# DenisKolodin/safe_gossip

Measured on AMD Instinct MI355X. Metric: node-rumor updates/sec (whole node) + % HBM roofline; rounds-to-full-spread, higher is better.
Workload: dtype u64

## Files before the change

include/safe_gossip.h:

```cpp
#ifndef SAFE_GOSSIP_H
#define SAFE_GOSSIP_H

#include <stdint.h>

#ifdef __cplusplus
extern "C" {
#endif

typedef enum {
    GS_OK = 0,
    GS_ERR_NO_PEERS = 1,
    GS_ERR_ALREADY_STARTED = 2,
    GS_ERR_SIG_FAILURE = 3,
    GS_ERR_IO = 4,
    GS_ERR_SERIALISATION = 5,
    GS_ERR_INVALID_ARGUMENT = -1,
    GS_ERR_UNSUPPORTED = -2,
    GS_ERR_HIP = -3,
    GS_ERR_OUT_OF_MEMORY = -4,
    GS_ERR_DEVICE_LIMIT = -5
} gs_status;

typedef enum { GS_SCHED_2P = 0, GS_SCHED_SEQ = 1 } gs_schedule;

typedef struct {
    uint32_t n_nodes;
    uint32_t n_rumors;
    uint64_t seed;
    uint32_t epoch;
    uint8_t counter_max;
    uint8_t max_c_rounds;
    uint8_t max_rounds;
    uint8_t schedule;
    int32_t device;
    uint32_t churn;
    uint32_t drop_push;
    uint32_t drop_pull;
    uint32_t rumor_slice;
    uint32_t reserved1[3];
} gs_config;

typedef struct {
    uint64_t rounds;
    uint64_t empty_pull_sent;
    uint64_t empty_push_sent;
    uint64_t full_message_sent;
    uint64_t full_message_received;
} gs_statistics_t;

typedef enum { GS_REDUCE_SUM = 0, GS_REDUCE_MIN = 1, GS_REDUCE_MAX = 2 } gs_reduce_op;

typedef struct {
    uint32_t round;
    uint32_t any_live;
} gs_round_report;

typedef struct gs_engine gs_engine;

#define GS_ABI_VERSION 2u
uint32_t    gs_abi_version(void);
const char *gs_build_id(void);

gs_status   gs_create(const gs_config *cfg, gs_engine **out);
void        gs_destroy(gs_engine *e);
gs_status   gs_get_params(const gs_engine *e, uint8_t out[3]);

gs_status   gs_send_new(gs_engine *e, uint32_t node, uint32_t rumor);

gs_status   gs_set_params(gs_engine *e, const uint8_t params[3]);

gs_status   gs_next_round(gs_engine *e, gs_round_report *report);

gs_status   gs_statistics(gs_engine *e, uint32_t node, gs_statistics_t *out);
gs_status   gs_statistics_all(gs_engine *e, uint64_t *out );
gs_status   gs_statistics_reduce(gs_engine *e, gs_reduce_op op, gs_statistics_t *out);
gs_status   gs_messages(gs_engine *e, uint32_t node, uint64_t *words );
gs_status   gs_known_all(gs_engine *e, uint64_t *words );
gs_status   gs_known_counts(gs_engine *e, uint64_t *known_total, uint64_t *nodes_complete);
gs_status   gs_known_counts_min(gs_engine *e, uint32_t min_known, uint64_t *known_total,
                                uint64_t *nodes_complete);
gs_status   gs_known_popcounts(gs_engine *e, uint32_t *counts);

gs_status   gs_dump_state(gs_engine *e, uint16_t *out);
gs_status   gs_dump_records(gs_engine *e, uint16_t *rec, uint32_t *psize);
gs_status   gs_state_digest(gs_engine *e, uint64_t *out);
gs_status   gs_state_digest_part(gs_engine *e, uint32_t rumor_lo, uint32_t words, uint64_t *dpart);
gs_status   gs_digest_finish(gs_engine *e, const uint64_t *dpart, uint32_t words, const uint64_t *stats,
                             uint64_t *out);

gs_status   gs_clear(gs_engine *e, uint32_t epoch);
gs_status   gs_sync(gs_engine *e);
uint32_t    gs_round(const gs_engine *e);

float       gs_last_round_kernel_ms(gs_engine *e);
void        gs_set_timing(gs_engine *e, int enable);
int32_t     gs_round_kernel_times(gs_engine *e, float *out_ms, uint32_t max);
double      gs_round_kernel_bytes(const gs_engine *e);
const char *gs_round_kernel_name(const gs_engine *e);
gs_status   gs_round_traffic(gs_engine *e, double *bytes_per_launch, uint32_t *launches);

gs_status   gs_shard_create(const gs_config *cfg, uint32_t rank, uint32_t world, gs_engine **out);
gs_status   gs_shard_create_parts(const gs_config *cfg, uint32_t rank, uint32_t world, uint32_t parts,
                                  gs_engine **out);
gs_status   gs_shard_info(const gs_engine *e, uint32_t info[14]);
gs_status   gs_shard_plan_info(const gs_config *cfg, uint32_t rank, uint32_t world, uint32_t parts,
                               uint32_t info[14]);
gs_status   gs_shard_bind(gs_engine *e, void *sendA0, void *sendA1, void *recvA0, void *recvA1,
                          void *sendB, void *recvB);
gs_status   gs_shard_round_part(gs_engine *e, uint32_t part);
gs_status   gs_shard_pull(gs_engine *e);
uint64_t    gs_stream(const gs_engine *e);
int         gs_device(const gs_engine *e);

gs_status   gs_slice_bind(gs_engine *e, void *buf0, void *buf1, void *buf2, void *obs);
gs_status   gs_slice_apply(gs_engine *e, uint32_t which);
gs_status   gs_slice_defer(gs_engine *e, uint32_t which);
gs_status   gs_slice_set_ext_limit(gs_engine *e, uint32_t limit);

#define GS_NET_ID_BYTES 128
typedef struct gs_net gs_net;
typedef enum { GS_NET_SLICES = 0, GS_NET_SHARDS = 1 } gs_net_mode;
gs_status   gs_net_unique_id(uint8_t id[GS_NET_ID_BYTES]);
gs_status   gs_net_create(const gs_config *cfg, gs_net_mode mode, uint32_t rank, uint32_t world, uint32_t parts,
                          const uint8_t id[GS_NET_ID_BYTES], gs_net **out);
gs_status   gs_net_create_local(const gs_config *cfg, gs_net_mode mode, uint32_t world, uint32_t parts,
                                gs_net **out);
void        gs_net_destroy(gs_net *net);
enum { GS_NET_U8 = 0, GS_NET_U32 = 1, GS_NET_U64 = 2 };
enum { GS_NET_SUM = 0, GS_NET_MIN = 1, GS_NET_MAX = 2 };
typedef struct {
    void *ctx;
    int (*alltoall)(void *ctx, const void *send, void *recv, uint64_t bytes_per_rank);
    int (*allreduce)(void *ctx, void *buf, uint64_t count, int dtype, int op);
    int (*allgather)(void *ctx, const void *send, void *recv, uint64_t bytes_per_rank);
} gs_net_collectives;
gs_status   gs_net_create_with(const gs_config *cfg, gs_net_mode mode, uint32_t rank, uint32_t world, uint32_t parts,
                               const gs_net_collectives *coll, gs_net **out);
gs_status   gs_net_send_new(gs_net *net, uint32_t node, uint32_t rumor);
gs_status   gs_net_next_round(gs_net *net, gs_round_report *report);
gs_status   gs_net_sync(gs_net *net);
gs_status   gs_net_clear(gs_net *net, uint32_t epoch);
gs_status   gs_net_known_counts(gs_net *net, uint64_t *known_total, uint64_t *nodes_complete);
gs_status   gs_net_statistics_all(gs_net *net, uint64_t *out );
gs_status   gs_net_dump_state(gs_net *net, uint16_t *out );
uint32_t    gs_net_local_engines(const gs_net *net);
gs_engine  *gs_net_engine(gs_net *net, uint32_t i);

gs_status   gs_rpc_encode(int pull, const uint8_t *msg, uint32_t msg_len, uint8_t counter, uint8_t *out,
                          uint32_t cap, uint32_t *out_len);
gs_status   gs_rpc_decode(const uint8_t *buf, uint32_t len, int *pull, uint32_t *msg_off, uint32_t *msg_len,
                          uint8_t *counter);
gs_status   gs_message_wrap(const uint8_t *payload, uint32_t len, const uint8_t signature[64], uint8_t *out,
                            uint32_t cap, uint32_t *out_len);
gs_status   gs_message_unwrap(const uint8_t *buf, uint32_t len, uint32_t *payload_off, uint32_t *payload_len,
                              uint32_t *signature_off);
gs_status   gs_set_rumor_key(gs_engine *e, uint32_t rumor, const uint8_t *key, uint32_t len);
gs_status   gs_rumor_key(const gs_engine *e, uint32_t rumor, uint8_t *out, uint32_t cap, uint32_t *len);
gs_status   gs_push_batch(gs_engine *e, uint32_t node, uint8_t *out, uint32_t cap, uint32_t *len,
                          uint32_t *count);
gs_status   gs_handle_received(gs_engine *e, uint32_t node, uint32_t peer, const uint8_t *msg,
                               uint32_t msg_len, uint8_t *out, uint32_t cap, uint32_t *out_len,
                               uint32_t *out_count);
gs_status   gs_handle_received_batch(gs_engine *e, uint32_t count, const uint32_t *nodes, const uint32_t *peers,
                                     const uint8_t *msgs, const uint32_t *off, const uint32_t *len, uint8_t *out,
                                     uint32_t cap, uint32_t *out_len, uint32_t *resp_off);

gs_status   gs_sha3_512(int device, uint32_t count, const uint8_t *data, const uint32_t *off,
                        const uint32_t *len, uint8_t *out);
gs_status   gs_ed25519_verify(int device, uint32_t count, const uint8_t *pubs, const uint8_t *sigs,
                              const uint8_t *msgs, const uint32_t *off, const uint32_t *len, uint8_t *ok);
gs_status   gs_ed25519_sign(int device, uint32_t count, const uint8_t *seeds, const uint8_t *msgs,
                            const uint32_t *off, const uint32_t *len, uint8_t *pubs, uint8_t *sigs);
gs_status   gs_handle_received_signed(gs_engine *e, uint32_t node, uint32_t peer, const uint8_t peer_key[32],
                                      const uint8_t node_seed[32], const uint8_t *msg, uint32_t msg_len,
                                      uint8_t *out, uint32_t cap, uint32_t *out_len, uint32_t *out_count);
gs_status   gs_push_batch_signed(gs_engine *e, uint32_t node, const uint8_t node_seed[32], uint8_t *out,
                                 uint32_t cap, uint32_t *len, uint32_t *count);

uint32_t    gs_peer(uint64_t seed, uint32_t epoch, uint32_t round, uint32_t node, uint32_t n);
uint32_t    gs_origin(uint64_t seed, uint32_t epoch, uint32_t rumor, uint32_t n);
uint32_t    gs_coin(uint64_t seed, uint32_t epoch, uint32_t round, uint32_t node);
uint32_t    gs_fault(uint64_t seed, uint32_t epoch, uint32_t round, uint32_t node,
// ... 9 lines not shown
```

safe_gossip_amd/__init__.py:

```python
from __future__ import annotations

import ctypes
import os
from dataclasses import dataclass
from typing import List, Optional, Sequence

import numpy as np

from .build import LIB_PATH

__all__ = [
    "Network", "Gossiper", "Statistics", "RoundReport", "GossipError", "NoPeers",
    "AlreadyStarted", "DeviceError", "derive_params", "peer_of", "origin_of", "coin_of",
    "send_messages", "load_library", "SYMBOLS", "rpc_encode", "rpc_decode", "message_wrap",
    "message_unwrap", "split_frames", "SigFailure", "sha3_512", "ed25519_sign", "ed25519_verify",
    "default_rumor_key",
]

class GossipError(Exception):

    code = None


class NoPeers(GossipError):
# ... 14 lines not shown
class DeviceError(GossipError):
    """Engine-side failure (no library, no GPU, HIP error, device limit)."""


_ERRORS = {1: NoPeers, 2: AlreadyStarted, 3: SigFailure}

class _Config(ctypes.Structure):
    _fields_ = [
        ("n_nodes", ctypes.c_uint32), ("n_rumors", ctypes.c_uint32),
        ("seed", ctypes.c_uint64), ("epoch", ctypes.c_uint32),
        ("counter_max", ctypes.c_uint8), ("max_c_rounds", ctypes.c_uint8),
        ("max_rounds", ctypes.c_uint8), ("schedule", ctypes.c_uint8),
        ("device", ctypes.c_int32), ("churn", ctypes.c_uint32),
        ("drop_push", ctypes.c_uint32), ("drop_pull", ctypes.c_uint32),
        ("rumor_slice", ctypes.c_uint32), ("reserved1", ctypes.c_uint32 * 3),
    ]


class _Stats(ctypes.Structure):
    _fields_ = [(f, ctypes.c_uint64) for f in (
        "rounds", "empty_pull_sent", "empty_push_sent", "full_message_sent",
        "full_message_received")]


class _Report(ctypes.Structure):
    _fields_ = [("round", ctypes.c_uint32), ("any_live", ctypes.c_uint32)]


_P = ctypes.c_void_p
_U8P = ctypes.POINTER(ctypes.c_uint8)
_U16P = ctypes.POINTER(ctypes.c_uint16)
_U32P = ctypes.POINTER(ctypes.c_uint32)
_U64P = ctypes.POINTER(ctypes.c_uint64)

SYMBOLS = {
    "gs_create": (ctypes.c_int, [ctypes.POINTER(_Config), ctypes.POINTER(_P)]),
    "gs_destroy": (None, [_P]),
    "gs_get_params": (ctypes.c_int, [_P, _U8P]),
    "gs_send_new": (ctypes.c_int, [_P, ctypes.c_uint32, ctypes.c_uint32]),
    "gs_next_round": (ctypes.c_int, [_P, ctypes.POINTER(_Report)]),
    "gs_statistics": (ctypes.c_int, [_P, ctypes.c_uint32, ctypes.POINTER(_Stats)]),
    "gs_statistics_all": (ctypes.c_int, [_P, _U64P]),
    "gs_statistics_reduce": (ctypes.c_int, [_P, ctypes.c_int, ctypes.POINTER(_Stats)]),
    "gs_messages": (ctypes.c_int, [_P, ctypes.c_uint32, _U64P]),
    "gs_known_all": (ctypes.c_int, [_P, _U64P]),
    "gs_known_counts": (ctypes.c_int, [_P, _U64P, _U64P]),
    "gs_known_counts_min": (ctypes.c_int, [_P, ctypes.c_uint32, _U64P, _U64P]),
    "gs_known_popcounts": (ctypes.c_int, [_P, _U32P]),
    "gs_set_params": (ctypes.c_int, [_P, _U8P]),
    "gs_rpc_encode": (ctypes.c_int, [ctypes.c_int, _U8P, ctypes.c_uint32, ctypes.c_uint8, _U8P,
                                     ctypes.c_uint32, _U32P]),
    "gs_rpc_decode": (ctypes.c_int, [_U8P, ctypes.c_uint32, ctypes.POINTER(ctypes.c_int), _U32P, _U32P,
                                     _U8P]),
    "gs_message_wrap": (ctypes.c_int, [_U8P, ctypes.c_uint32, _U8P, _U8P, ctypes.c_uint32, _U32P]),
    "gs_message_unwrap": (ctypes.c_int, [_U8P, ctypes.c_uint32, _U32P, _U32P, _U32P]),
    "gs_set_rumor_key": (ctypes.c_int, [_P, ctypes.c_uint32, _U8P, ctypes.c_uint32]),
    "gs_rumor_key": (ctypes.c_int, [_P, ctypes.c_uint32, _U8P, ctypes.c_uint32, _U32P]),
    "gs_push_batch": (ctypes.c_int, [_P, ctypes.c_uint32, _U8P, ctypes.c_uint32, _U32P, _U32P]),
    "gs_handle_received": (ctypes.c_int, [_P, ctypes.c_uint32, ctypes.c_uint32, _U8P, ctypes.c_uint32,
                                          _U8P, ctypes.c_uint32, _U32P, _U32P]),
    "gs_handle_received_batch": (ctypes.c_int, [_P, ctypes.c_uint32, _U32P, _U32P, _U8P, _U32P, _U32P, _U8P,
                                                ctypes.c_uint32, _U32P, _U32P]),
    "gs_device": (ctypes.c_int, [_P]),
    "gs_sha3_512": (ctypes.c_int, [ctypes.c_int, ctypes.c_uint32, _U8P, _U32P, _U32P, _U8P]),
    "gs_ed25519_verify": (ctypes.c_int, [ctypes.c_int, ctypes.c_uint32, _U8P, _U8P, _U8P, _U32P, _U32P, _U8P]),
    "gs_ed25519_sign": (ctypes.c_int, [ctypes.c_int, ctypes.c_uint32, _U8P, _U8P, _U32P, _U32P, _U8P, _U8P]),
    "gs_handle_received_signed": (ctypes.c_int, [_P, ctypes.c_uint32, ctypes.c_uint32, _U8P, _U8P, _U8P,
                                                 ctypes.c_uint32, _U8P, ctypes.c_uint32, _U32P, _U32P]),
    "gs_push_batch_signed": (ctypes.c_int, [_P, ctypes.c_uint32, _U8P, _U8P, ctypes.c_uint32, _U32P, _U32P]),
    "gs_dump_state": (ctypes.c_int, [_P, _U16P]),
    "gs_dump_records": (ctypes.c_int, [_P, _U16P, _U32P]),
    "gs_state_digest": (ctypes.c_int, [_P, _U64P]),
    "gs_state_digest_part": (ctypes.c_int, [_P, ctypes.c_uint32, ctypes.c_uint32, ctypes.c_void_p]),
    "gs_digest_finish": (ctypes.c_int, [_P, ctypes.c_void_p, ctypes.c_uint32, _U64P, _U64P]),
    "gs_clear": (ctypes.c_int, [_P, ctypes.c_uint32]),
    "gs_sync": (ctypes.c_int, [_P]),
    "gs_round": (ctypes.c_uint32, [_P]),
    "gs_last_round_kernel_ms": (ctypes.c_float, [_P]),
    "gs_set_timing": (None, [_P, ctypes.c_int]),
    "gs_round_kernel_times": (ctypes.c_int32, [_P, ctypes.POINTER(ctypes.c_float), ctypes.c_uint32]),
    "gs_round_kernel_bytes": (ctypes.c_double, [_P]),
    "gs_round_kernel_name": (ctypes.c_char_p, [_P]),
    "gs_round_traffic": (ctypes.c_int, [_P, ctypes.POINTER(ctypes.c_double), _U32P]),
    "gs_peer": (ctypes.c_uint32, [ctypes.c_uint64, ctypes.c_uint32, ctypes.c_uint32,
                                  ctypes.c_uint32, ctypes.c_uint32]),
    "gs_origin": (ctypes.c_uint32, [ctypes.c_uint64, ctypes.c_uint32, ctypes.c_uint32,
                                    ctypes.c_uint32]),
    "gs_coin": (ctypes.c_uint32, [ctypes.c_uint64, ctypes.c_uint32, ctypes.c_uint32,
                                  ctypes.c_uint32]),
    "gs_fault": (ctypes.c_uint32, [ctypes.c_uint64, ctypes.c_uint32, ctypes.c_uint32,
                                   ctypes.c_uint32, ctypes.c_uint32, ctypes.c_uint32,
                                   ctypes.c_uint32]),
    "gs_derive_params": (None, [ctypes.c_uint32, _U8P]),
    "gs_status_string": (ctypes.c_char_p, [ctypes.c_int]),
    "gs_abi_version": (ctypes.c_uint32, []),
    "gs_build_id": (ctypes.c_char_p, []),
    "gs_shard_create": (ctypes.c_int, [ctypes.POINTER(_Config), ctypes.c_uint32, ctypes.c_uint32,
                                       ctypes.POINTER(_P)]),
    "gs_shard_create_parts": (ctypes.c_int, [ctypes.POINTER(_Config), ctypes.c_uint32, ctypes.c_uint32,
                                             ctypes.c_uint32, ctypes.POINTER(_P)]),
    "gs_shard_round_part": (ctypes.c_int, [_P, ctypes.c_uint32]),
    "gs_shard_info": (ctypes.c_int, [_P, _U32P]),
    "gs_shard_plan_info": (ctypes.c_int, [_P, ctypes.c_uint32, ctypes.c_uint32, ctypes.c_uint32, _U32P]),
    "gs_shard_bind": (ctypes.c_int, [_P, _P, _P, _P, _P, _P, _P]),
    "gs_shard_pull": (ctypes.c_int, [_P]),
    "gs_stream": (ctypes.c_uint64, [_P]),
    "gs_slice_bind": (ctypes.c_int, [_P, _P, _P, _P, _P]),
    "gs_slice_apply": (ctypes.c_int, [_P, ctypes.c_uint32]),
    "gs_slice_defer": (ctypes.c_int, [_P, ctypes.c_uint32]),
    "gs_slice_set_ext_limit": (ctypes.c_int, [_P, ctypes.c_uint32]),
    "gs_net_unique_id": (ctypes.c_int, [_U8P]),
    "gs_net_create": (ctypes.c_int, [_P, ctypes.c_int, ctypes.c_uint32, ctypes.c_uint32, ctypes.c_uint32, _U8P,
                                     ctypes.POINTER(_P)]),
    "gs_net_create_local": (ctypes.c_int, [_P, ctypes.c_int, ctypes.c_uint32, ctypes.c_uint32, ctypes.POINTER(_P)]),
    "gs_net_create_with": (ctypes.c_int, [_P, ctypes.c_int, ctypes.c_uint32, ctypes.c_uint32, ctypes.c_uint32, _P,
                                          ctypes.POINTER(_P)]),
    "gs_net_destroy": (None, [_P]),
    "gs_net_send_new": (ctypes.c_int, [_P, ctypes.c_uint32, ctypes.c_uint32]),
    "gs_net_next_round": (ctypes.c_int, [_P, _P]),
    "gs_net_sync": (ctypes.c_int, [_P]),
    "gs_net_clear": (ctypes.c_int, [_P, ctypes.c_uint32]),
    "gs_net_known_counts": (ctypes.c_int, [_P, _U64P, _U64P]),
    "gs_net_statistics_all": (ctypes.c_int, [_P, _U64P]),
    "gs_net_dump_state": (ctypes.c_int, [_P, _U16P]),
    "gs_net_local_engines": (ctypes.c_uint32, [_P]),
    "gs_net_engine": (_P, [_P, ctypes.c_uint32]),
}

_LIB = None


def _share_torch_hip_runtime() -> None:
    if os.environ.get("SAFE_GOSSIP_AMD_HIP_RUNTIME") == "system":
        return
    import importlib.util
    spec = importlib.util.find_spec("torch")
    if spec is None or not spec.origin:
        return
    rt = os.path.join(os.path.dirname(spec.origin), "lib", "libamdhip64.so")
    if os.path.exists(rt):
        ctypes.CDLL(rt, mode=ctypes.RTLD_GLOBAL)


ABI_VERSION = 2


def build_id() -> str:
    return load_library().gs_build_id().decode()


def load_library(path: Optional[str] = None):
    global _LIB
    if _LIB is not None and path is None:
        return _LIB
    p = path or os.environ.get("SAFE_GOSSIP_AMD_LIB", LIB_PATH)
    if not os.path.exists(p):
        raise DeviceError(f"engine library not built: {p} (run __graft_entry__.build())")
    _share_torch_hip_runtime()
    lib = ctypes.CDLL(p)
    for name, (res, args) in SYMBOLS.items():
        fn = getattr(lib, name)
        fn.restype = res
        fn.argtypes = args
    if lib.gs_abi_version() != ABI_VERSION:
        raise DeviceError(f"{p}: C ABI version {lib.gs_abi_version()}, this binding speaks {ABI_VERSION}")
    from .build import source_hash
# ... 391 lines not shown

    def handle_received_batch(self, rpcs) -> List[List[bytes]]:
        return engine_handle_received_batch(self._lib, self._h, rpcs)

    def handle_received_signed(self, node: int, peer: int, peer_key: bytes, message: bytes,
                               node_seed: Optional[bytes] = None) -> List[bytes]:
        assert len(peer_key) == 32 and (node_seed is None or len(node_seed) == 32)
        cap = 4096
        while True:
            out = (ctypes.c_uint8 * cap)()
            n, c = ctypes.c_uint32(), ctypes.c_uint32()
            st = self._lib.gs_handle_received_signed(self._h, node, peer, _buf(peer_key),
                                                     _buf(node_seed) if node_seed else None, _buf(message),
                                                     len(message), out, cap, ctypes.byref(n), ctypes.byref(c))
            if st == 5 and n.value > cap:
                cap = n.value
                continue
            _check(st)
            return split_frames(bytes(out)[:n.value])

    def push_batch_signed(self, node: int, node_seed: bytes) -> List[bytes]:
        assert len(node_seed) == 32
        n, c = ctypes.c_uint32(), ctypes.c_uint32()
        self._lib.gs_push_batch_signed(self._h, node, _buf(node_seed), None, 0, ctypes.byref(n), ctypes.byref(c))
        out = (ctypes.c_uint8 * max(1, n.value))()
        _check(self._lib.gs_push_batch_signed(self._h, node, _buf(node_seed), out, n.value, ctypes.byref(n),
                                              ctypes.byref(c)))
        return split_frames(bytes(out)[:n.value])

    def known_popcounts(self) -> np.ndarray:
        out = np.zeros(self.n, dtype=np.uint32)
        _check(self._lib.gs_known_popcounts(self._h, out.ctypes.data_as(_U32P)))
        return out

    def dump_state(self) -> np.ndarray:
        out = np.zeros((self.n, self.R), dtype=np.uint16)
        _check(self._lib.gs_dump_state(self._h, out.ctypes.data_as(_U16P)))
        return out

    def dump_records(self):
        rec = np.zeros((self.n, self.R), dtype=np.uint16)
        ps = np.zeros(self.n, dtype=np.uint32)
        _check(self._lib.gs_dump_records(self._h, rec.ctypes.data_as(_U16P),
                                         ps.ctypes.data_as(_U32P)))
        return rec, ps

    def state_digest(self) -> np.ndarray:
        out = np.zeros(self.n, dtype=np.uint64)
        _check(self._lib.gs_state_digest(self._h, out.ctypes.data_as(_U64P)))
        return out

    def clear(self, epoch: Optional[int] = None) -> None:
        self.epoch = self.epoch + 1 if epoch is None else epoch
        _check(self._lib.gs_clear(self._h, self.epoch))

    def sync(self) -> None:
        _check(self._lib.gs_sync(self._h))

    def set_timing(self, on: bool) -> None:
        self._lib.gs_set_timing(self._h, 1 if on else 0)

    def last_round_kernel_ms(self) -> float:
        return float(self._lib.gs_last_round_kernel_ms(self._h))

    def round_kernel_times(self, max_n: int = 4096) -> np.ndarray:
        out = np.zeros(max_n, dtype=np.float32)
        m = self._lib.gs_round_kernel_times(self._h, out.ctypes.data_as(ctypes.POINTER(ctypes.c_float)),
                                            max_n)
        if m < 0:
            raise DeviceError("kernel timing unavailable")
        return out[:m]

    def round_kernel_bytes(self) -> float:
        return float(self._lib.gs_round_kernel_bytes(self._h))

    def round_kernel_name(self) -> str:
        return self._lib.gs_round_kernel_name(self._h).decode()

    def round_traffic(self):
        b, m = ctypes.c_double(), ctypes.c_uint32()
        _check(self._lib.gs_round_traffic(self._h, ctypes.byref(b), ctypes.byref(m)))
        return float(b.value), int(m.value)


class Gossiper:

    def __init__(self, net: Network, node: int):
        self._net = net
        self._node = node

    def id(self) -> int:
        return self._node

    def send_new(self, rumor: int) -> None:
        self._net.send_new(self._node, rumor)

    def messages(self) -> List[int]:
        return self._net.messages(self._node)

    def statistics(self) -> Statistics:
        return self._net.statistics(self._node)

    def push_batch(self) -> List[bytes]:
        return self._net.push_batch(self._node)

    def handle_received_message(self, peer: int, message: bytes) -> List[bytes]:
        return self._net.handle_received(self._node, peer, message)


def send_messages(net: Network, num_of_msgs: int):
    assert num_of_msgs >= 1
    if num_of_msgs > net.R:
        raise ValueError(f"num_of_msgs {num_of_msgs} > rumor slots {net.R}")
    n = net.n
    next_rumor = 0
    net.send_new(origin_of(net.seed, net.epoch, 0, n), next_rumor)
    next_rumor += 1
    processed = True
    rounds_run = 0
    round_full = 0
    while processed:
        rnd = net.round + 1
        if next_rumor < num_of_msgs:
            for x in range(n):
                if next_rumor >= num_of_msgs:
                    break
                if coin_of(net.seed, net.epoch, rnd, x):
                    net.send_new(x, next_rumor)
                    next_rumor += 1
        rep = net.next_round()
        processed = rep.any_live
        rounds_run += 1
        if not round_full and next_rumor == num_of_msgs:
            _, complete = net.known_counts(num_of_msgs)
            if complete == n:
                round_full = net.round
    tot = net.statistics_reduce("sum")
    stats = Statistics(net.statistics(n - 1).rounds, tot.empty_pull_sent - n,
                       tot.empty_push_sent - n, tot.full_message_sent, tot.full_message_received)
    counts = net.known_popcounts().astype(np.int64)
    missed = counts < num_of_msgs
    nodes_missed = int(missed.sum())
    msgs_missed = int((num_of_msgs - counts[missed]).sum())
    net.clear()
    return nodes_missed, msgs_missed, stats, rounds_run, round_full
```

safe_gossip_amd/csrc/gs_common.h:

```cpp
#pragma once
#include <hip/hip_runtime.h>
#include <stdint.h>

namespace gs {

typedef unsigned long long u64;

constexpr uint32_t kPhM0 = 0xD2511F53u, kPhM1 = 0xCD9E8D57u;
constexpr uint32_t kPhW0 = 0x9E3779B9u, kPhW1 = 0xBB67AE85u;

constexpr uint32_t kStreamPeer = 0, kStreamOrigin = 1, kStreamCoin = 2, kStreamFault = 3;

__host__ __device__ __forceinline__ uint32_t mulhi32(uint32_t a, uint32_t b) {
#if defined(__HIP_DEVICE_COMPILE__)
    return __umulhi(a, b);
#else
    return (uint32_t)(((uint64_t)a * b) >> 32);
#endif
}

struct Ph4 {
    uint32_t w0, w1, w2, w3;
};

// ... 30 lines not shown
}

__host__ __device__ __forceinline__ uint32_t peer_of(uint64_t seed, uint32_t epoch,
                                                    uint32_t round, uint32_t node, uint32_t n) {
    uint32_t u = mulhi64(philox_u64(round, node, kStreamPeer, epoch, seed), n - 1u);
    return u + (u >= node ? 1u : 0u);
}

__host__ __device__ __forceinline__ uint32_t origin_of(uint64_t seed, uint32_t epoch,
                                                      uint32_t rumor, uint32_t n) {
    return mulhi64(philox_u64(rumor, 0u, kStreamOrigin, epoch, seed), n);
}

__host__ __device__ __forceinline__ uint32_t coin_of(uint64_t seed, uint32_t epoch,
                                                    uint32_t round, uint32_t node) {
    return (uint32_t)(philox_u64(round, node, kStreamCoin, epoch, seed) & 1u);
}

struct Faults {
    uint32_t churn, push, pull;
};

__host__ __device__ __forceinline__ bool faults_on(const Faults &f) {
    return (f.churn | f.push | f.pull) != 0u;
}

__host__ __device__ __forceinline__ bool offline_of(uint64_t seed, uint32_t epoch, uint32_t round,
                                                   uint32_t node, uint32_t churn) {
    return churn != 0u && philox4(round, node, kStreamFault, epoch, seed).w0 < churn;
}

constexpr uint32_t kTgDead = 1u << 31;
constexpr uint32_t kTgNoPull = 1u << 30;
constexpr uint32_t kTgOff = 1u << 29;
constexpr uint32_t kTgMask = kTgOff - 1u;

constexpr uint32_t kSeqGot = 0x80u, kSeqDep = 0x40u, kSeqLevelMask = 0x3Fu;
constexpr uint32_t kSeqInline = kSeqLevelMask;

__host__ __device__ __forceinline__ uint32_t target_word(uint64_t seed, uint32_t epoch,
                                                        uint32_t round, uint32_t node, uint32_t n,
                                                        const Faults &f) {
    const uint32_t t = peer_of(seed, epoch, round, node, n);
    if (!faults_on(f)) return t;
    const Ph4 w = philox4(round, node, kStreamFault, epoch, seed);
    if (w.w0 < f.churn) return t | kTgDead | kTgNoPull | kTgOff;
    if (w.w1 < f.push || offline_of(seed, epoch, round, t, f.churn)) return t | kTgDead | kTgNoPull;
    if (w.w2 < f.pull) return t | kTgNoPull;
    return t;
}

constexpr int kPlanes = 8;
constexpr int kClsPlanes = 3;

struct Geometry {
    uint32_t n;
    uint32_t R;
    uint32_t rpad;
    uint32_t W;
    uint32_t small;
    uint32_t lognpu;
    uint32_t logr;
    uint64_t units;
    uint64_t nseg;
};

constexpr uint32_t kInline = 3;
constexpr uint32_t kSibInline = 3;
constexpr uint32_t kSerialMask = 0xFFFFFFu;
constexpr uint32_t kMaxIn = 30;
constexpr uint32_t kExtCopiesMax = 96;
constexpr int kVoteBits = 5, kVoteBitsExt = 7;
constexpr uint32_t kFirstShift = 5;
struct alignas(16) InRec {
    uint32_t kf, s[kInline];
    __host__ __device__ uint32_t k() const { return kf & ((1u << kFirstShift) - 1u); }
    __host__ __device__ uint32_t first() const { return kf >> kFirstShift; }
};
struct alignas(16) SibRec {
    uint32_t tag, e[kSibInline];
};
constexpr uint32_t kInSkipShift = 28;
constexpr uint32_t kInFlagMask = (1u << kInSkipShift) - 1u;
constexpr uint32_t kSibSkipShift = 5;
constexpr uint32_t kSkipBit = 1u << 31;
constexpr uint32_t kIdMask = kSkipBit - 1u;
constexpr uint32_t kSibZNeed = 1u << 7;
constexpr uint32_t kSibRankMask = 0x1Fu;

constexpr uint32_t kDlvInline = 2;
constexpr uint32_t kDlvNoZ = 31u;
constexpr uint32_t kDlvMetaNoPull = 10u, kDlvMetaOff = 11u;
static_assert(kTgNoPull == 1u << 30 && kTgOff == 1u << 29, "meta flag bits mirror the target-word flags");
constexpr uint32_t kDlvFirstShift = 12u;
struct alignas(4) DlvRec {
    uint32_t mf, c[kDlvInline];
};
static_assert(sizeof(DlvRec) == 12, "one delivery record is 12 bytes");

__host__ __device__ inline u64 digest_mix(u64 z) {
    z = (z ^ (z >> 30)) * 0xBF58476D1CE4E5B9ull;
    z = (z ^ (z >> 27)) * 0x94D049BB133111EBull;
    return z ^ (z >> 31);
}
__host__ __device__ inline u64 digest_plane_k(uint32_t p) { return 0x9E3779B97F4A7C15ull * (2ull * p + 1ull); }
__host__ __device__ inline void digest_planes(u64 m, u64 B, u64 C, u64 D, u64 crB, u64 crC, u64 a0, u64 a1,
                                              const u64 *bp, u64 anyC, const u64 *c1, const u64 *c2, u64 pl[20]) {
    const u64 BC = B | C, E = B | crB;
    pl[0] = crB | B | D;
    pl[1] = crC | C | D;
    pl[2] = crB | (BC & a0);
    pl[3] = BC & a1;
    for (int i = 0; i < 5; ++i) pl[4 + i] = BC & bp[i];
    pl[9] = E & anyC;
    for (int i = 0; i < 5; ++i) {
        pl[10 + i] = E & c1[i];
        pl[15 + i] = E & c2[i];
    }
    for (int p = 0; p < 20; ++p) pl[p] &= m;
}
__host__ __device__ inline u64 digest_sum(const u64 pl[20], uint32_t shl = 0) {
    u64 h = 0;
    for (uint32_t p = 0; p < 20; ++p) h += (pl[p] << shl) * digest_plane_k(p);
    return h;
}
__host__ __device__ inline u64 digest_fin(uint32_t j, u64 h) { return digest_mix(h ^ digest_mix((u64)j + 0x632BE59BD9B4E019ull)); }
__host__ __device__ inline u64 digest_word(uint32_t j, u64 m, u64 B, u64 C, u64 D, u64 crB, u64 crC, u64 a0,
                                           u64 a1, const u64 *bp, u64 anyC, const u64 *c1, const u64 *c2) {
    u64 pl[20];
    digest_planes(m, B, C, D, crB, crC, a0, a1, bp, anyC, c1, c2, pl);
    return digest_fin(j, digest_sum(pl));
}
__host__ __device__ inline u64 digest_node(uint32_t psize, const u64 *st5) {
    u64 h = digest_mix((1ull << 63) | psize);
    for (int i = 0; i < 5; ++i) h += digest_mix(st5[i] ^ (0x9E3779B97F4A7C15ull * (u64)(i + 1)));
    return h;
}

}
```

safe_gossip_amd/csrc/gs_device.h:

```cpp
#pragma once
#include "gs_common.h"

namespace gs {

#define GS_DEV __device__ __forceinline__

GS_DEV uint32_t popc(u64 v) { return (uint32_t)__popcll(v); }

GS_DEV void zero_for_build(uint32_t *buf, uint32_t words, u64 *one) {
    const uint32_t gt = blockIdx.x * blockDim.x + threadIdx.x;
    for (uint32_t i = gt; i < words; i += gridDim.x * blockDim.x) buf[i] = 0u;
    if (one && gt == 0u) *one = 0ull;
}

GS_DEV void add5(u64 (&c)[5], u64 in) {
#pragma unroll
    for (int i = 0; i < 5; ++i) {
        u64 t = c[i] & in;
        c[i] ^= in;
        in = t;
    }
}

template <int NB>
GS_DEV u64 ge_k(const u64 (&x)[NB], uint32_t K) {
    u64 b = 0ull;
#pragma unroll
    for (int i = 0; i < NB; ++i) {
        const uint32_t m = 0u - ((K >> i) & 1u);
        const u64 k = ((u64)m << 32) | m;
        b = (~x[i] & b) | (k & (~x[i] | b));
    }
    return K >= (1u << NB) ? 0ull : ~b;
}

template <int NB>
GS_DEV u64 ge_u(const u64 (&x)[NB], uint32_t K) {
    if (K >= (1u << NB)) return 0ull;
    u64 b = 0ull;
#pragma unroll
    for (int i = 0; i < NB; ++i) {
        const u64 k = ((K >> i) & 1u) ? ~0ull : 0ull;
        b = (~x[i] & b) | (k & (~x[i] | b));
    }
    return ~b;
}

template <typename T>
GS_DEV uint32_t popcT(T v) {
    if constexpr (sizeof(T) == 8) return (uint32_t)__popcll(v);
    else return (uint32_t)__popc(v);
}
template <int NB, typename T>
GS_DEV void addcT(T (&c)[NB], T in) {
#pragma unroll
    for (int i = 0; i < NB; ++i) {
        const T t = c[i] & in;
        c[i] ^= in;
        in = t;
    }
}
template <int NB, typename T>
GS_DEV T ge_uT(const T (&x)[NB], uint32_t K) {
    if (K >= (1u << NB)) return (T)0;
    T b = 0;
#pragma unroll
    for (int i = 0; i < NB; ++i) {
        const T k = ((K >> i) & 1u) ? (T)~(T)0 : (T)0;
        b = (~x[i] & b) | (k & (~x[i] | b));
    }
    return ~b;
}
template <int NB, typename T>
GS_DEV T ge_kT(const T (&x)[NB], uint32_t K) {
    T b = 0;
#pragma unroll
    for (int i = 0; i < NB; ++i) {
        const T k = (T)0 - (T)((K >> i) & 1u);
        b = (~x[i] & b) | (k & (~x[i] | b));
    }
    return K >= (1u << NB) ? (T)0 : ~b;
}

template <typename T>
struct ClsT {
    T c, a0, a1;
};
using Cls = ClsT<u64>;

#ifndef GS_CLS_VEC
#define GS_CLS_VEC 0
// ... 200 lines not shown
```

safe_gossip_amd/csrc/gs_engine.cpp:

```cpp
#include "../../include/safe_gossip.h"

#include <hip/hip_runtime.h>

#include <algorithm>
#include <cmath>
#include <cstdio>
#include <cstdlib>
#include <cstring>
#include <map>
#include <set>
#include <string>
#include <tuple>
#include <utility>
#include <vector>

#include "gs_common.h"
#include "gs_kernels.h"

using gs::u64;

struct gs_engine {
    gs::Geometry g{};
    uint64_t seed = 0;
    uint32_t epoch = 0;
    gs::Faults faults{};
    bool seq = false;
    u64 *Wb = nullptr;
    uint8_t *sinfo = nullptr;
    uint32_t *seqw = nullptr;
    uint32_t seq_round = ~0u;
    u64 *pend = nullptr;
    uint32_t *offc = nullptr;
    uint8_t cmax = 0, maxc = 0, maxr = 0;
    int device = 0;
    hipStream_t stream = nullptr;
    u64 *S[2] = {nullptr, nullptr};
    int cur = 0;
    struct CsrSet {
        uint32_t *src = nullptr, *tg = nullptr, *scratch = nullptr, *region = nullptr;
        gs::InRec *IN8 = nullptr;
        gs::SibRec *SIB8 = nullptr;
        gs::DlvRec *DR = nullptr;
        uint32_t *pull = nullptr;
        u64 *zl = nullptr;
        uint32_t serial = 0;
        uint32_t wraps = 0;
    } csr[2];
    uint32_t serial_wraps = 0;
    bool filt = false;
    u64 *lvm = nullptr, *cpm = nullptr;
    u64 *rows_dev = nullptr;
    uint32_t filt_launches = 0;
    bool dlv = false;
    uint32_t dlv_pack = 1;
    bool w32 = false;
    u64 *acct = nullptr;
    uint32_t *pc = nullptr;
    uint16_t *kn = nullptr;
    hipStream_t cstream = nullptr;
    uint32_t build_serial = 0;
    uint32_t *flags = nullptr;
    gs::CsrPlan plan{};
    bool shard = false;
    uint32_t n_global = 0;
    bool slice = false;
    uint8_t *eb[4] = {nullptr, nullptr, nullptr, nullptr};
    int eb_defer = -1;
    gs::ShardPlan sp{};
    gs::ShardPlanLayout spl{};
    gs::ShardEdgeLayout sel{};
    uint32_t *planw[3] = {nullptr, nullptr, nullptr};
    uint32_t *edgew[2] = {nullptr, nullptr};
    hipEvent_t ev_plan[3] = {nullptr, nullptr, nullptr};
    hipEvent_t ev_edges[2] = {nullptr, nullptr};
    hipEvent_t ev_main = nullptr;
    u64 *sendA[2] = {nullptr, nullptr}, *recvA[2] = {nullptr, nullptr};
    u64 *sendB = nullptr, *recvB = nullptr;
    uint32_t pulled_round = 0;
    uint32_t parts_done = 0;
    gs::RoundArgs ra{};
    int ra_mode = 0;
    bool ra_prezeroed = false;
    uint32_t *st32 = nullptr;
    bool st16 = false;
    u64 *st64 = nullptr;
    uint32_t *live = nullptr;
    uint32_t fold_every = 1, since_fold = 0;
    u64 *inj_key = nullptr, *inj_mask = nullptr;
    u64 *inj_host = nullptr;
    uint32_t inj_cap = 0;
    std::vector<std::pair<uint32_t, uint32_t>> pending;
    std::vector<std::string> keys;
    std::map<std::string, uint32_t> key_rumor;
    std::vector<uint32_t> key_order;
    struct Ext {
        uint32_t node, seq, info, peer;
    };
    std::vector<Ext> ext;
    std::set<std::pair<uint32_t, uint32_t>> ext_peers;
    std::map<uint32_t, uint32_t> ext_fp;
    std::set<std::tuple<uint32_t, uint32_t, uint32_t>> ext_copy_peers;
    std::map<std::pair<uint32_t, uint32_t>, uint32_t> ext_copies;
    uint32_t ext_limit = 0;
    u64 *ext_dev = nullptr;
    uint32_t ext_cap = 0, ext_uploaded = 0;
    uint16_t *node_state = nullptr;
    uint32_t *batch_lists = nullptr;
    uint16_t *batch_codes = nullptr;
    size_t batch_lists_cap = 0, batch_codes_cap = 0;
    uint32_t round = 0;
    bool deliver_pending = false;
    u64 *obs_known = nullptr, *obs_stats = nullptr, *partials = nullptr;
    uint16_t *obs_state = nullptr, *obs_rec = nullptr;
    uint32_t *obs_psize = nullptr;
    u64 *obs_digest = nullptr;
    u64 *obs_pend = nullptr;
    uint32_t obs_pend_cap = 0;
    bool obs_valid = false;
    bool started = false;
    hipEvent_t lt0 = nullptr, lt1 = nullptr;
    bool timing = false, timed = false;
    std::vector<hipEvent_t> tev;
    std::vector<uint8_t> tparts;
    uint32_t tcount = 0;
    uint32_t tslot = ~0u;
};

namespace {

constexpr uint32_t kReduceBlocks = 1024;
constexpr uint32_t kTimingSlots = 4096;

void report_hip(hipError_t err, const char *what, int line) {
    static const bool on = [] {
        const char *v = std::getenv("SAFE_GOSSIP_AMD_DEBUG");
        return v && *v && *v != '0';
    }();
    if (on) std::fprintf(stderr, "safe_gossip_amd: %s failed at gs_engine.cpp:%d: %s\n", what, line,
                         hipGetErrorString(err));
}
#define GS_HIP(expr)                                   \
    do {                                               \
        hipError_t _e = (expr);                        \
        if (_e != hipSuccess) {                        \
            report_hip(_e, #expr, __LINE__);           \
            return GS_ERR_HIP;                         \
        }                                              \
    } while (0)

uint32_t next_pow2(uint32_t v) {
    uint32_t p = 1;
    while (p < v) p <<= 1;
    return p;
}
uint32_t ilog2(uint32_t v) {
    uint32_t l = 0;
    while ((1u << l) < v) ++l;
    return l;
}

gs_status set_device(gs_engine *e) {
    return hipSetDevice(e->device) == hipSuccess ? GS_OK : GS_ERR_HIP;
}

template <typename T>
hipError_t dalloc(T **p, size_t count) {
    return hipMalloc((void **)p, std::max<size_t>(count, 1) * sizeof(T));
}

void release(gs_engine *e) {
    if (!e) return;
    (void)hipSetDevice(e->device);
    if (e->stream) (void)hipStreamSynchronize(e->stream);
    if (e->cstream) (void)hipStreamSynchronize(e->cstream);
    for (auto &c : e->csr) {
        void *cb[] = {c.src, c.tg, c.scratch, c.region, c.IN8, c.SIB8, c.DR, c.pull, c.zl};
        for (void *b : cb)
            if (b) (void)hipFree(b);
    }
    for (int i = 0; i < 3; ++i) {
        if (e->planw[i]) (void)hipFree(e->planw[i]);
        if (e->ev_plan[i]) (void)hipEventDestroy(e->ev_plan[i]);
    }
    for (int i = 0; i < 2; ++i) {
        if (e->edgew[i]) (void)hipFree(e->edgew[i]);
        if (e->ev_edges[i]) (void)hipEventDestroy(e->ev_edges[i]);
    }
    if (e->ev_main) (void)hipEventDestroy(e->ev_main);
    if (e->cstream) (void)hipStreamDestroy(e->cstream);
    void *bufs[] = {e->lvm, e->cpm, e->rows_dev, e->acct, e->pc, e->kn, e->Wb, e->sinfo, e->seqw, e->pend, e->offc, e->S[0], e->S[1], e->flags, e->live, e->st32, e->st64, e->inj_key, e->inj_mask, e->obs_known, e->obs_stats,
                    e->partials, e->obs_state, e->obs_rec, e->obs_psize, e->obs_digest, e->obs_pend, e->ext_dev,
                    e->node_state, e->batch_lists, e->batch_codes};
    for (void *b : bufs)
        if (b) (void)hipFree(b);
    if (e->inj_host) (void)hipHostFree(e->inj_host);
    for (hipEvent_t ev : e->tev) (void)hipEventDestroy(ev);
    if (e->stream) (void)hipStreamDestroy(e->stream);
    delete e;
}

gs_status reset_state(gs_engine *e) {
    const gs::Geometry &g = e->g;
    GS_HIP(hipStreamSynchronize(e->cstream));
    const size_t sw = (size_t)g.units * gs::kPlanes * g.W;
    GS_HIP(hipMemsetAsync(e->S[0], 0, sw * sizeof(u64), e->stream));
    GS_HIP(hipMemsetAsync(e->S[1], 0, sw * sizeof(u64), e->stream));
    GS_HIP(hipMemsetAsync(e->st32, 0, (size_t)4 * g.n * sizeof(uint32_t), e->stream));
    GS_HIP(hipMemsetAsync(e->st64, 0, (size_t)4 * g.n * sizeof(u64), e->stream));
    if (e->offc) GS_HIP(hipMemsetAsync(e->offc, 0, (size_t)g.n * sizeof(uint32_t), e->stream));
    e->since_fold = 0;
    GS_HIP(hipMemsetAsync(e->flags, 0, 4 * sizeof(uint32_t), e->stream));
    GS_HIP(hipMemsetAsync(e->live, 0, (size_t)2 * gs::kLiveSlots * gs::kLiveStride * sizeof(uint32_t), e->stream));
    if (e->dlv) {
        size_t first = 0, words = 0;
        gs::inlist_cfill_range(e->plan, &first, &words);
        for (auto &c : e->csr)
            if (words && c.scratch) GS_HIP(hipMemsetAsync(c.scratch + first, 0, words * sizeof(uint32_t), e->stream));
    }
    e->cur = 0;
    e->round = 0;
    e->eb_defer = -1;
    e->seq_round = ~0u;
    e->pulled_round = 0;
    e->parts_done = 0;
    e->deliver_pending = false;
    e->pending.clear();
    e->obs_valid = false;
    e->started = false;
    e->ext.clear();
    e->ext_peers.clear();
    e->ext_fp.clear();
    e->ext_copy_peers.clear();
    e->ext_copies.clear();
    e->ext_uploaded = 0;
    return GS_OK;
}

gs_status upload_ext(gs_engine *e) {
    const uint32_t m = (uint32_t)e->ext.size();
    if (m == e->ext_uploaded) return GS_OK;
    if (m > e->ext_cap) {
        GS_HIP(hipStreamSynchronize(e->stream));
        if (e->ext_dev) (void)hipFree(e->ext_dev);
        e->ext_dev = nullptr;
        e->ext_cap = 0;
        const uint32_t cap = std::max<uint32_t>(1024, 2 * m);
        GS_HIP(dalloc(&e->ext_dev, cap));
        e->ext_cap = cap;
    }
    std::vector<gs_engine::Ext> v(e->ext);
    std::stable_sort(v.begin(), v.end(), [](const gs_engine::Ext &a, const gs_engine::Ext &b) {
        return a.node != b.node ? a.node < b.node : a.seq < b.seq;
    });
    std::vector<u64> keys(m);
    for (uint32_t i = 0; i < m; ++i) keys[i] = ((u64)v[i].node << 32) | v[i].info;
    GS_HIP(hipStreamSynchronize(e->stream));
    GS_HIP(hipMemcpyAsync(e->ext_dev, keys.data(), m * sizeof(u64), hipMemcpyHostToDevice, e->stream));
    GS_HIP(hipStreamSynchronize(e->stream));
    e->ext_uploaded = m;
    return GS_OK;
}

gs_status device_limit(gs_engine *e) {
    uint32_t fl = 0;
    GS_HIP(hipStreamSynchronize(e->cstream));
    GS_HIP(hipMemcpyAsync(&fl, e->flags + 2, sizeof(uint32_t), hipMemcpyDeviceToHost, e->stream));
    GS_HIP(hipStreamSynchronize(e->stream));
    return fl ? GS_ERR_DEVICE_LIMIT : GS_OK;
}

gs::RoundArgs base_args(gs_engine *e) {
    gs::RoundArgs a{};
    a.Scur = e->S[e->cur];
    a.Snext = e->S[e->cur ^ 1];
    if (e->dlv) gs::dlv_tail_parts(e->plan, &a.dlv_tlog, &a.dlv_tper);
    if (e->shard) {
        const uint32_t t = e->round;
        uint32_t *cur = e->planw[t % 3], *nxt = e->planw[(t + 1) % 3], *ed = e->edgew[t % 2];
        a.IN = reinterpret_cast<const uint4 *>(ed + e->sel.IN);
        a.IN2 = ed + e->sel.IN2;
        a.src = ed + e->sel.EP;
        a.spos_cur = cur + e->spl.SPOSB;
        a.spos_next = nxt + e->spl.SPOSA;
        a.tg = cur + e->spl.tg;
        a.node_lo = e->sp.lo;
        a.tg_next = nxt + e->spl.tg;
        a.recvA = e->recvA[t % 2];
        a.recvB = e->recvB;
        a.sendA = e->sendA[(t + 1) % 2];
        a.sp = gs::ShardRows{e->sp.G,  e->sp.P,   e->sp.W,     e->sp.capP,  e->sp.idrows,
                             e->sp.rw, e->sp.rwb, e->sp.codes, e->sp.chunk, e->sp.n};
        if (e->dlv) {
            a.DR = e->csr[0].DR;
            a.dtail = e->csr[0].src;
            a.recvA_next = e->recvA[(t + 1) % 2];
        }
    } else {
        const auto &cs = e->csr[e->round & 1u];
        a.IN8 = cs.IN8;
        a.SIB8 = cs.SIB8;
        a.DR = cs.DR;
        a.dtail = e->dlv ? cs.src : nullptr;
        a.pull = cs.pull;
        a.pc_out = e->pc;
        a.kn_out = e->kn;
        a.src = cs.src;
        a.tg = cs.tg;
        a.serial = cs.serial;
        if (e->filt) {
            a.zlm = cs.zl;
            a.lvm = e->lvm;
            a.cpm = e->cpm;
        }
    }
    a.st32 = e->st32;
    a.st16 = e->st16 ? 1u : 0u;
    a.st64 = e->st64;
    a.f = e->faults;
    a.pend = e->pend;
    a.offc = e->offc;
    if (e->seq) {
        a.Wb = e->Wb;
        a.sinfo = e->sinfo;
    }
    a.obs_rounds = e->round;
    a.flags = e->flags;
    a.live = e->live;
    if (e->deliver_pending && !e->ext.empty()) {
        a.ext = e->ext_dev;
        a.n_ext = e->ext_uploaded;
    }
    a.obs_only = 0xFFFFFFFFu;
    a.dlv_pack = e->dlv_pack;
    a.w32 = e->w32 ? 1u : 0u;
    a.g = e->g;
    a.seed = e->seed;
    a.epoch = e->epoch;
    a.round_new = e->round + 1;
    a.cmax = e->cmax;
    a.maxc = e->maxc;
    a.maxr = e->maxr;
    return a;
}

gs_status upload_injections(gs_engine *e, uint32_t *n_inj) {
    *n_inj = 0;
    if (e->pending.empty()) return GS_OK;
    const gs::Geometry &g = e->g;
    std::vector<std::pair<u64, u64>> km;
    km.reserve(e->pending.size());
    for (auto &p : e->pending) {
        const uint32_t x = p.first, r = p.second;
        if (g.small) km.emplace_back((u64)x, 1ull << r);
        else km.emplace_back((u64)x * g.W + (r >> 6), 1ull << (r & 63));
    }
    std::sort(km.begin(), km.end());
    std::vector<std::pair<u64, u64>> merged;
    for (auto &v : km) {
        if (!merged.empty() && merged.back().first == v.first) merged.back().second |= v.second;
        else merged.push_back(v);
    }
    const uint32_t m = (uint32_t)merged.size();
    if (m > e->inj_cap) {
        GS_HIP(hipStreamSynchronize(e->stream));
        if (e->inj_key) (void)hipFree(e->inj_key);
        if (e->inj_mask) (void)hipFree(e->inj_mask);
        if (e->inj_host) (void)hipHostFree(e->inj_host);
        e->inj_key = e->inj_mask = e->inj_host = nullptr;
        uint32_t cap = std::max<uint32_t>(m, 1024);
        GS_HIP(dalloc(&e->inj_key, cap));
        GS_HIP(dalloc(&e->inj_mask, cap));
        GS_HIP(hipHostMalloc((void **)&e->inj_host, 2 * (size_t)cap * sizeof(u64), 0));
        e->inj_cap = cap;
    }
    GS_HIP(hipStreamSynchronize(e->stream));
    for (uint32_t i = 0; i < m; ++i) {
        e->inj_host[i] = merged[i].first;
        e->inj_host[e->inj_cap + i] = merged[i].second;
    }
    GS_HIP(hipMemcpyAsync(e->inj_key, e->inj_host, m * sizeof(u64), hipMemcpyHostToDevice, e->stream));
    GS_HIP(hipMemcpyAsync(e->inj_mask, e->inj_host + e->inj_cap, m * sizeof(u64),
                          hipMemcpyHostToDevice, e->stream));
    e->pending.clear();
    *n_inj = m;
    return GS_OK;
}

gs_status ensure_obs(gs_engine *e, bool dumps) {
    const gs::Geometry &g = e->g;
    const uint32_t KW = (g.R + 63) / 64;
    if (!e->obs_known) {
        GS_HIP(dalloc(&e->obs_known, (size_t)g.n * KW));
        GS_HIP(dalloc(&e->obs_stats, (size_t)g.n * 5));
        GS_HIP(dalloc(&e->partials, (size_t)kReduceBlocks * 5));
        GS_HIP(dalloc(&e->obs_psize, (size_t)g.n));
// ... 227 lines not shown
    if (!cfg || !out) return GS_ERR_INVALID_ARGUMENT;
    *out = nullptr;
    gs::ShardPlan sp{};
    uint8_t p[3];
    const gs_status cst = check_config(cfg, rank, world, parts, &sp, p);
    if (cst != GS_OK) return cst;
    const uint32_t nglob = cfg->n_nodes, R = cfg->n_rumors;
    const uint32_t n = world ? sp.m : nglob;

    gs_engine *e = new gs_engine();
    e->shard = world != 0;
    e->slice = cfg->rumor_slice != 0;
    e->n_global = nglob;
    e->sp = sp;
    e->seed = cfg->seed;
    e->epoch = cfg->epoch;
    e->faults = gs::Faults{cfg->churn, cfg->drop_push, cfg->drop_pull};
    e->seq = cfg->schedule == GS_SCHED_SEQ;
    e->cmax = p[0];
    e->maxc = p[1];
    e->maxr = p[2];
    int dev = cfg->device;
    if (dev < 0 && hipGetDevice(&dev) != hipSuccess) {
        delete e;
        return GS_ERR_HIP;
    }
    e->device = dev;
    if (hipSetDevice(dev) != hipSuccess) {
        delete e;
        return GS_ERR_HIP;
    }
    gs::Geometry &g = e->g;
    g.n = n;
    g.R = R;
    g.rpad = next_pow2(R);
    g.logr = ilog2(g.rpad);
    if (g.rpad >= 64) {
        g.small = 0;
        g.W = g.rpad / 64;
        g.lognpu = 0;
        g.units = n;
        g.nseg = (uint64_t)n * g.W;
    } else {
        g.small = 1;
        g.W = 1;
        g.lognpu = 6 - g.logr;
        const uint64_t npu = 1ull << g.lognpu;
        g.units = (n + npu - 1) / npu;
        g.nseg = n;
    }
    {
        const char *v = std::getenv("SAFE_GOSSIP_AMD_NO_DLV");
        const bool off = v && *v && *v != '0';
        e->dlv = e->shard ? e->sp.codes != 0
                          : !off && !e->seq && g.small && g.rpad <= 16 && gs::dlv_plan(n).binned;
    }
    {
        const char *v = std::getenv("SAFE_GOSSIP_AMD_DLV_PACK");
        const std::string m = v ? v : "";
        e->dlv_pack = m == "0" ? 0u : (m == "u64" ? 2u : (m == "u32x1" ? 3u : 1u));
    }
    e->plan = e->dlv ? gs::dlv_plan(e->shard ? std::max(n, shard_keys(e->sp)) : n) : gs::csr_plan(n);
    if (e->dlv && !e->plan.binned) {
        delete e;
        return GS_ERR_UNSUPPORTED;
    }
    e->keys.resize(R);
    e->key_order.resize(R);
    for (uint32_t r = 0; r < R; ++r) {
        const char k[12] = {4, 0, 0, 0, 0, 0, 0, 0, (char)(r >> 24), (char)(r >> 16), (char)(r >> 8), (char)r};
        e->keys[r] = std::string(k, 12);
        e->key_rumor[e->keys[r]] = r;
        e->key_order[r] = r;
    }
    {
        const char *w = std::getenv("SAFE_GOSSIP_AMD_W32");
        e->w32 = (w && *w) ? *w != '0' : (e->g.small && e->g.rpad == 32u);
    }
    {
        const char *v = std::getenv("SAFE_GOSSIP_AMD_FILTER");
        const bool off = v && *v == '0';
        e->filt = !off && !e->shard && !e->seq && !e->dlv && e->plan.binned && (g.small || g.W <= 8);
    }
    e->st16 = e->dlv;
    e->fold_every = (uint32_t)std::max<uint64_t>(1, (e->st16 ? 0xFFFFull : 0xFFFFFFFFull) / (32ull * g.rpad + 32) / 2);
    bool ok;
    if (e->shard) {
        int least = 0, greatest = 0;
        ok = hipDeviceGetStreamPriorityRange(&least, &greatest) == hipSuccess &&
             hipStreamCreateWithPriority(&e->stream, hipStreamNonBlocking, greatest) == hipSuccess &&
             hipStreamCreateWithPriority(&e->cstream, hipStreamNonBlocking, least) == hipSuccess;
    } else {
        ok = hipStreamCreateWithFlags(&e->stream, hipStreamNonBlocking) == hipSuccess &&
             hipStreamCreateWithFlags(&e->cstream, hipStreamNonBlocking) == hipSuccess;
    }
    for (int i = 0; i < 3 && ok && e->shard; ++i) {
        const size_t words = gs::shard_plan_words(e->sp, &e->spl);
        ok = hipEventCreateWithFlags(&e->ev_plan[i], hipEventDisableTiming) == hipSuccess &&
             dalloc(&e->planw[i], words) == hipSuccess;
    }
    for (int i = 0; i < 2 && ok && e->shard && !e->dlv; ++i) {
        const size_t words = gs::shard_edge_words(e->sp, &e->sel);
        ok = hipEventCreateWithFlags(&e->ev_edges[i], hipEventDisableTiming) == hipSuccess &&
             dalloc(&e->edgew[i], words) == hipSuccess &&
             hipMemsetAsync(e->edgew[i], 0, words * sizeof(uint32_t), e->stream) == hipSuccess;
    }
    if (ok && e->shard) ok = hipEventCreateWithFlags(&e->ev_main, hipEventDisableTiming) == hipSuccess;
    if (ok && e->shard && e->dlv) {
        const gs::InListSizes dz = gs::inlist_sizes(e->plan);
        auto &c = e->csr[0];
        ok = dalloc(&c.src, dz.src_words) == hipSuccess && dalloc(&c.region, dz.region_words) == hipSuccess &&
             dalloc(&c.scratch, dz.scratch_words) == hipSuccess && dalloc(&c.DR, e->plan.n) == hipSuccess;
    }
    const gs::InListSizes isz = gs::inlist_sizes(e->plan);
    const size_t npad = gs::tile_padded(n);
    const size_t sw_pad = (size_t)gs::tile_padded(g.units) * gs::kPlanes * g.W;
    for (int i = 0; i < 2 && ok && !e->shard; ++i) {
        auto &c = e->csr[i];
        ok = dalloc(&c.src, isz.src_words) == hipSuccess && dalloc(&c.tg, npad) == hipSuccess &&
             dalloc(&c.region, isz.region_words) == hipSuccess &&
             dalloc(&c.scratch, isz.scratch_words) == hipSuccess &&
             hipMemsetAsync(c.scratch, 0, std::max<size_t>(isz.scratch_words, 1) * sizeof(uint32_t), e->stream) == hipSuccess;
        if (ok && e->dlv) {
            ok = dalloc(&c.DR, n) == hipSuccess && dalloc(&c.pull, n) == hipSuccess;
        } else if (ok) {
            ok = dalloc(&c.IN8, npad) == hipSuccess && dalloc(&c.SIB8, npad) == hipSuccess &&
                 hipMemsetAsync(c.SIB8, 0, std::max<size_t>(n, 1) * sizeof(gs::SibRec), e->stream) == hipSuccess;
            if (ok && e->filt) ok = dalloc(&c.zl, gs::node_map_words(n)) == hipSuccess;
        }
    }
    ok = ok && dalloc(&e->S[0], sw_pad) == hipSuccess && dalloc(&e->S[1], sw_pad) == hipSuccess &&
         dalloc(&e->flags, 4) == hipSuccess && dalloc(&e->live, (size_t)2 * gs::kLiveSlots * gs::kLiveStride) == hipSuccess && dalloc(&e->st32, (size_t)4 * npad) == hipSuccess &&
         dalloc(&e->st64, (size_t)4 * n) == hipSuccess;
    if (ok && e->dlv) ok = dalloc(&e->pc, n) == hipSuccess && (e->shard || dalloc(&e->kn, n) == hipSuccess);
    if (ok && e->filt)
        ok = dalloc(&e->lvm, gs::node_map_words(n)) == hipSuccess &&
             dalloc(&e->cpm, gs::node_map_words(n)) == hipSuccess &&
             dalloc(&e->rows_dev, 2) == hipSuccess &&
             dalloc(&e->acct, 1) == hipSuccess && hipMemsetAsync(e->acct, 0, sizeof(u64), e->stream) == hipSuccess;
    if (ok && e->seq)
        ok = dalloc(&e->Wb, (size_t)n * 2 * g.W) == hipSuccess && dalloc(&e->sinfo, n) == hipSuccess &&
             dalloc(&e->seqw, (size_t)gs::seq_blocks(n) * gs::kSeqLists + gs::kSeqLists + n) == hipSuccess;
    if (ok && e->faults.churn)
        ok = dalloc(&e->pend, (size_t)n * 2 * g.W) == hipSuccess && dalloc(&e->offc, n) == hipSuccess;
    if (!ok) {
        hipError_t le = hipGetLastError();
        release(e);
        return le == hipErrorOutOfMemory ? GS_ERR_OUT_OF_MEMORY : GS_ERR_HIP;
    }
    if (reset_state(e) != GS_OK || hipStreamSynchronize(e->stream) != hipSuccess) {
        release(e);
        return GS_ERR_HIP;
    }
    *out = e;
    return GS_OK;
}

gs_status launch_plan(gs_engine *e, uint32_t r) {
    GS_HIP(gs::launch_shard_plan(e->sp, e->spl, e->planw[r % 3], e->sendA[(e->dlv ? r : r + 1) % 2], e->seed,
                                 e->epoch, r, e->faults, e->flags, e->cstream));
    GS_HIP(hipEventRecord(e->ev_plan[r % 3], e->cstream));
    return GS_OK;
}

gs_status launch_edges(gs_engine *e, uint32_t r) {
    GS_HIP(gs::launch_shard_edges(e->sp, e->sel, e->edgew[r % 2], e->recvA[(r + 1) % 2],
                                  e->planw[r % 3] + e->spl.tg, e->seed, e->epoch, r, e->faults, e->flags,
                                  e->cstream));
    GS_HIP(hipEventRecord(e->ev_edges[r % 2], e->cstream));
    return GS_OK;
}

gs_status shard_build(gs_engine *e) {
    const uint32_t t = e->round;
    GS_HIP(hipEventRecord(e->ev_main, e->stream));
    GS_HIP(hipStreamWaitEvent(e->cstream, e->ev_main, 0));
    gs_status st = launch_plan(e, t + 2);
    if (st != GS_OK) return st;
    e->pulled_round = t;
    auto &c = e->csr[0];
    gs::InListArgs la{};
    la.p = e->plan;
    la.dlv = 1;
    la.S = e->S[e->cur];
    la.g = e->g;
    la.DR = c.DR;
    la.dtail = c.src;
    la.src = c.src;
    la.region = c.region;
    la.scratch = c.scratch;
    la.flags = e->flags;
    la.seed = e->seed;
    la.epoch = e->epoch;
    la.round = t;
    la.f = e->faults;
    la.rowsA = reinterpret_cast<const uint32_t *>(e->recvA[t % 2]);
    la.pullB = reinterpret_cast<uint32_t *>(e->sendB);
    la.sr = gs::ShardRows{e->sp.G,  e->sp.P,   e->sp.W,     e->sp.capP,  e->sp.idrows,
                          e->sp.rw, e->sp.rwb, e->sp.codes, e->sp.chunk, e->sp.n};
    la.nkeys = shard_keys(e->sp);
    la.ntargets = e->g.n;
    la.self_rank = e->sp.g;
    la.self_cnt = e->planw[t % 3] + e->spl.cnt + (size_t)e->sp.g * e->sp.P;
    la.pullB_self = reinterpret_cast<uint32_t *>(e->recvB);
    GS_HIP(gs::launch_build_inlists(la, e->stream));
    return GS_OK;
}

}

extern "C" {

gs_status gs_create(const gs_config *cfg, gs_engine **out) { return create_engine(cfg, 0, 0, 0, out); }

gs_status gs_shard_create(const gs_config *cfg, uint32_t rank, uint32_t world, gs_engine **out) {
    if (world == 0) return GS_ERR_INVALID_ARGUMENT;
    return create_engine(cfg, rank, world, 1, out);
}

gs_status gs_shard_create_parts(const gs_config *cfg, uint32_t rank, uint32_t world, uint32_t parts,
                                gs_engine **out) {
    if (world == 0) return GS_ERR_INVALID_ARGUMENT;
// ... 107 lines not shown
    return GS_OK;
}

}

namespace {

gs_status next_serial(gs_engine *e, gs_engine::CsrSet &c, hipStream_t bs) {
    c.serial = ++e->build_serial & gs::kSerialMask;
    if (c.serial == 0) {
        ++e->serial_wraps;
        c.serial = ++e->build_serial & gs::kSerialMask;
    }
    if (c.wraps != e->serial_wraps) {
        if (c.SIB8) GS_HIP(hipMemsetAsync(c.SIB8, 0, (size_t)e->g.n * sizeof(gs::SibRec), bs));
        c.wraps = e->serial_wraps;
    }
    return GS_OK;
}

gs::InListArgs inlist_args(gs_engine *e, gs_engine::CsrSet &c, uint32_t round) {
    gs::InListArgs la{};
    la.p = e->plan;
    la.tg = c.tg;
    la.IN8 = c.IN8;
    la.SIB8 = c.SIB8;
    la.src = c.src;
    la.region = c.region;
    la.scratch = c.scratch;
    la.flags = e->flags;
    la.serial = c.serial;
    la.seed = e->seed;
    la.epoch = e->epoch;
    la.round = round;
    la.f = e->faults;
    if (e->filt) {
        la.lvm = e->lvm;
        la.cpm = e->cpm;
        la.zl = c.zl;
        la.rows = e->rows_dev + (round & 1u);
    }
    if (e->dlv) {
        la.dlv = 1;
        la.S = e->S[e->cur];
        la.PC = e->pc;
        la.KN = e->kn;
        la.g = e->g;
        la.DR = c.DR;
        la.dtail = c.src;
        la.pull = c.pull;
    }
    return la;
}

gs_status round_begin(gs_engine *e) {
    gs_status st = GS_OK;
    if (e->shard) {
        GS_HIP(hipEventRecord(e->ev_main, e->stream));
        GS_HIP(hipStreamWaitEvent(e->cstream, e->ev_main, 0));
        if (e->round == 0) {
            st = launch_plan(e, 1);
            if (st != GS_OK) return st;
        }
    }
    uint32_t n_inj = 0;
    st = upload_injections(e, &n_inj);
    if (st == GS_OK && e->deliver_pending) st = upload_ext(e);
    if (st != GS_OK) return st;
    gs::RoundArgs a = base_args(e);
    a.inj_key = e->inj_key;
    a.inj_mask = e->inj_mask;
    a.n_inj = n_inj;
    const uint32_t R0 = e->round;
    if (e->slice) {
        a.emin = e->eb[(R0 + 1u) % 3u];
        if (e->eb_defer >= 0) a.eadd = e->eb[e->eb_defer];
        e->eb_defer = -1;
    }
    if (e->filt && e->deliver_pending && e->timing) {
        a.acct = e->acct;
        a.rows_cnt = e->rows_dev + (R0 & 1u);
        e->filt_launches++;
    }
    if (e->shard) {
        GS_HIP(hipStreamWaitEvent(e->stream, e->ev_plan[(R0 + 1) % 3], 0));
        if (e->deliver_pending && !e->dlv) GS_HIP(hipStreamWaitEvent(e->stream, e->ev_edges[R0 % 2], 0));
    } else if (e->deliver_pending) {
        st = seq_prepare(e);
        if (st != GS_OK) return st;
    }
    e->ra_prezeroed = !e->shard;
    if (e->ra_prezeroed) {
        auto &c = e->csr[(R0 + 1u) & 1u];
        size_t first = 0, words = 0;
        gs::inlist_zero_range(e->plan, &first, &words);
        if (words) {
            a.zero_buf = c.scratch + first;
            a.zero_words = (uint32_t)words;
        }
        if (e->filt) a.zero_rows = e->rows_dev + ((R0 + 1u) & 1u);
        gs::inlist_cfill_range(e->plan, &first, &words);
        if (words) {
            a.zero_buf2 = e->csr[R0 & 1u].scratch + first;
            a.zero_words2 = (uint32_t)words;
        }
    }
    e->ra = a;
    e->ra_mode = e->deliver_pending ? 1 : 0;
    e->tslot = ~0u;
    if (e->timing && e->tcount < kTimingSlots) {
        e->tslot = e->tcount++;
        e->tparts[e->tslot] = 0;
    }
    return GS_OK;
}

uint32_t dlv_nodes_per_lane(const gs_engine *e) {
    if (e->dlv_pack == 3) return 1u;
    if (e->g.rpad < 16) return 4u;
    return e->dlv_pack == 2 ? 4u : 2u;
}

gs_status launch_part(gs_engine *e, uint32_t h) {
    gs::RoundArgs a = e->ra;
    if (e->shard && e->sp.P > 1) {
        const u64 bn = e->dlv ? 256ull * dlv_nodes_per_lane(e) : 256ull;
        const u64 nblk = e->dlv ? ((u64)e->g.n + bn - 1) / bn : (e->g.nseg + 255) / 256;
        const u64 per = e->dlv ? (u64)e->sp.mP / bn : e->g.small ? (u64)e->sp.bP : (u64)e->sp.mP * e->g.W / 256;
        const u64 b0 = std::min<u64>((u64)h * per, nblk), b1 = std::min<u64>(b0 + per, nblk);
        if (b1 == b0) return GS_OK;
        a.blk_off = (uint32_t)b0;
        a.blk_count = (uint32_t)(b1 - b0);
    }
    hipEvent_t t0 = nullptr, t1 = nullptr;
    if (e->timing && e->tslot != ~0u) {
        t0 = e->tev[2 * ((size_t)e->tslot * gs::kMaxParts + h)];
        t1 = e->tev[2 * ((size_t)e->tslot * gs::kMaxParts + h) + 1];
        if (!e->tparts[e->tslot]) e->lt0 = t0;
        e->tparts[e->tslot] |= (uint8_t)(1u << h);
        e->lt1 = t1;
    }
    if (t0) GS_HIP(hipEventRecord(t0, e->stream));
    GS_HIP(gs::launch_round(a, e->ra_mode, e->stream));
    if (t1) GS_HIP(hipEventRecord(t1, e->stream));
    return GS_OK;
}

gs_status round_end(gs_engine *e, gs_round_report *report) {
    gs_status st = GS_OK;
    const uint32_t R0 = e->round;
    e->timed = e->timing;
    e->round += 1;
    e->cur ^= 1;
    e->deliver_pending = true;
    e->ext.clear();
    e->ext_peers.clear();
    e->ext_fp.clear();
    e->ext_copy_peers.clear();
    e->ext_copies.clear();
    e->ext_uploaded = 0;
    e->obs_valid = false;
    if (++e->since_fold >= e->fold_every) {
        GS_HIP(gs::launch_stats_fold(e->st32, e->st64, e->g.n, e->st16 ? 1u : 0u, e->stream));
        e->since_fold = 0;
    }
    if (e->shard) {
        if (R0 == 0) {
            st = launch_plan(e, 2);
            if (st != GS_OK) return st;
        }
        GS_HIP(hipStreamWaitEvent(e->stream, e->ev_plan[(R0 + 2) % 3], 0));
    } else {
        auto &c = e->csr[e->round & 1u];
        st = next_serial(e, c, e->stream);
        if (st != GS_OK) return st;
        gs::InListArgs la = inlist_args(e, c, e->round);
        la.prezeroed = e->ra_prezeroed ? 1u : 0u;
        GS_HIP(gs::launch_build_inlists(la, e->stream));
    }
    if (report) {
        uint32_t fl[4];
        static thread_local uint32_t lw[gs::kLiveSlots * gs::kLiveStride];
        GS_HIP(hipMemcpyAsync(fl, e->flags, sizeof(fl), hipMemcpyDeviceToHost, e->stream));
        GS_HIP(hipMemcpyAsync(lw, e->live + (size_t)(e->round & 1u) * gs::kLiveSlots * gs::kLiveStride, sizeof(lw),
                              hipMemcpyDeviceToHost, e->stream));
        GS_HIP(hipStreamSynchronize(e->stream));
        report->round = e->round;
        uint32_t any = 0;
        for (uint32_t i = 0; i < gs::kLiveSlots; ++i) any |= lw[i * gs::kLiveStride];
        report->any_live = any;
        if (fl[2]) return GS_ERR_DEVICE_LIMIT;
    }
    return GS_OK;
}

gs_status round_checks(gs_engine *e) {
    if ((e->shard ? e->n_global : e->g.n) < 2) return GS_ERR_NO_PEERS;
    if (e->shard && !e->sendB) return GS_ERR_INVALID_ARGUMENT;
    if (e->slice && !e->eb[0]) return GS_ERR_INVALID_ARGUMENT;
    if (e->shard && e->round > 0 && e->pulled_round != e->round) return GS_ERR_INVALID_ARGUMENT;
    return set_device(e);
}

}

extern "C" {

gs_status gs_shard_round_part(gs_engine *e, uint32_t part) {
    if (!e || !e->shard || part != e->parts_done || part >= e->sp.P) return GS_ERR_INVALID_ARGUMENT;
    gs_status st = round_checks(e);
    if (st == GS_OK && part == 0) st = round_begin(e);
    if (st == GS_OK) st = launch_part(e, part);
    if (st != GS_OK) {
        e->parts_done = 0;
        return st;
    }
    e->parts_done = part + 1;
    return GS_OK;
}

gs_status gs_next_round(gs_engine *e, gs_round_report *report) {
    if (!e) return GS_ERR_INVALID_ARGUMENT;
    gs_status st = round_checks(e);
    if (st == GS_OK && e->parts_done == 0) st = round_begin(e);
    const uint32_t parts = e->shard ? e->sp.P : 1u;
    for (uint32_t h = e->parts_done; st == GS_OK && h < parts; ++h) st = launch_part(e, h);
// ... 158 lines not shown
    if (!e->pending.empty()) return GS_ERR_INVALID_ARGUMENT;
    gs_status st = set_device(e);
    if (st == GS_OK) st = observe(e, false, true);
    if (st != GS_OK) return st;
    GS_HIP(hipMemcpy(out, e->obs_digest, (size_t)e->g.n * sizeof(u64), hipMemcpyDeviceToHost));
    return GS_OK;
}

gs_status gs_state_digest_part(gs_engine *e, uint32_t rumor_lo, uint32_t words, uint64_t *dpart) {
    if (!e || !dpart || words == 0 || (uint64_t)rumor_lo + e->g.R > 64ull * words) return GS_ERR_INVALID_ARGUMENT;
    if (!e->pending.empty()) return GS_ERR_INVALID_ARGUMENT;
    gs_status st = set_device(e);
    if (st == GS_OK) st = observe(e, false, false, reinterpret_cast<u64 *>(dpart), rumor_lo, words);
    if (st != GS_OK) return st;
    GS_HIP(hipStreamSynchronize(e->stream));
    return GS_OK;
}

gs_status gs_digest_finish(gs_engine *e, const uint64_t *dpart, uint32_t words, const uint64_t *stats,
                           uint64_t *out) {
    if (!e || !dpart || !stats || !out || words == 0) return GS_ERR_INVALID_ARGUMENT;
    if (!e->obs_psize) return GS_ERR_INVALID_ARGUMENT;
    gs_status st = set_device(e);
    if (st != GS_OK) return st;
    if (!e->obs_digest) GS_HIP(dalloc(&e->obs_digest, e->g.n));
    GS_HIP(hipMemcpyAsync(e->obs_stats, stats, (size_t)e->g.n * 5 * sizeof(u64), hipMemcpyHostToDevice, e->stream));
    GS_HIP(gs::launch_digest_finish(reinterpret_cast<const u64 *>(dpart), e->g.n, words, e->obs_psize, e->obs_stats,
                                    e->obs_digest, e->stream));
    GS_HIP(hipMemcpyAsync(out, e->obs_digest, (size_t)e->g.n * sizeof(u64), hipMemcpyDeviceToHost, e->stream));
    GS_HIP(hipStreamSynchronize(e->stream));
    e->obs_valid = false;
    return GS_OK;
}

gs_status gs_dump_records(gs_engine *e, uint16_t *rec, uint32_t *psize) {
    if (!e || !rec) return GS_ERR_INVALID_ARGUMENT;
    gs_status st = set_device(e);
    if (st == GS_OK) st = observe(e, true);
    if (st != GS_OK) return st;
    GS_HIP(hipMemcpy(rec, e->obs_rec, (size_t)e->g.n * e->g.R * sizeof(uint16_t), hipMemcpyDeviceToHost));
    if (psize)
        GS_HIP(hipMemcpy(psize, e->obs_psize, (size_t)e->g.n * sizeof(uint32_t), hipMemcpyDeviceToHost));
    return GS_OK;
}

gs_status gs_clear(gs_engine *e, uint32_t epoch) {
    if (!e) return GS_ERR_INVALID_ARGUMENT;
    gs_status st = set_device(e);
    if (st != GS_OK) return st;
    const gs_status lim = device_limit(e);
    if (lim != GS_OK && lim != GS_ERR_DEVICE_LIMIT) return lim;
    e->epoch = epoch;
    st = reset_state(e);
    if (st != GS_OK) return st;
    GS_HIP(hipStreamSynchronize(e->stream));
    return lim;
}

gs_status gs_sync(gs_engine *e) {
    if (!e) return GS_ERR_INVALID_ARGUMENT;
    gs_status st = set_device(e);
    if (st != GS_OK) return st;
    GS_HIP(hipStreamSynchronize(e->stream));
    GS_HIP(hipStreamSynchronize(e->cstream));
    return device_limit(e);
}

void gs_set_timing(gs_engine *e, int enable) {
    if (!e) return;
    e->timing = enable != 0;
    if (e->timing && e->tev.empty()) {
        (void)hipSetDevice(e->device);
        e->tev.resize(2 * (size_t)kTimingSlots * gs::kMaxParts, nullptr);
        e->tparts.assign(kTimingSlots, 0);
        for (auto &ev : e->tev)
            if (hipEventCreateWithFlags(&ev, hipEventDisableSystemFence) != hipSuccess) {
                e->timing = false;
                return;
            }
    }
    e->tcount = 0;
    if (e->timing && e->filt) {
        (void)hipSetDevice(e->device);
        if (hipMemsetAsync(e->acct, 0, sizeof(u64), e->stream) == hipSuccess) e->filt_launches = 0;
    }
}

int32_t gs_round_kernel_times(gs_engine *e, float *out_ms, uint32_t max) {
    if (!e || !out_ms) return -1;
    if (hipStreamSynchronize(e->stream) != hipSuccess) return -1;
    const uint32_t m = std::min(max, e->tcount);
    for (uint32_t i = 0; i < m; ++i) {
        float sum = 0.0f;
        for (uint32_t h = 0; h < gs::kMaxParts; ++h) {
            if (!(e->tparts[i] & (1u << h))) continue;
            const size_t k = 2 * ((size_t)i * gs::kMaxParts + h);
            float ms = -1.0f;
            if (hipEventElapsedTime(&ms, e->tev[k], e->tev[k + 1]) != hipSuccess) return -1;
            sum += ms;
        }
        out_ms[i] = sum;
    }
    e->tcount = 0;
    return (int32_t)m;
}

float gs_last_round_kernel_ms(gs_engine *e) {
    if (!e || !e->timed || !e->lt0 || !e->lt1) return -1.0f;
    if (hipEventSynchronize(e->lt1) != hipSuccess) return -1.0f;
    float ms = -1.0f;
    if (hipEventElapsedTime(&ms, e->lt0, e->lt1) != hipSuccess) return -1.0f;
    return ms;
}

gs_status gs_set_rumor_key(gs_engine *e, uint32_t rumor, const uint8_t *key, uint32_t len) {
    if (!e || (len && !key) || rumor >= e->g.R) return GS_ERR_INVALID_ARGUMENT;
    const std::string k(reinterpret_cast<const char *>(key), len);
    auto it = e->key_rumor.find(k);
    if (it != e->key_rumor.end()) return it->second == rumor ? GS_OK : GS_ERR_INVALID_ARGUMENT;
    e->key_rumor.erase(e->keys[rumor]);
    e->keys[rumor] = k;
    e->key_rumor[k] = rumor;
    std::sort(e->key_order.begin(), e->key_order.end(),
              [e](uint32_t x, uint32_t y) { return e->keys[x] < e->keys[y]; });
    return GS_OK;
}

gs_status gs_rumor_key(const gs_engine *e, uint32_t rumor, uint8_t *out, uint32_t cap, uint32_t *len) {
    if (!e || !len || rumor >= e->g.R) return GS_ERR_INVALID_ARGUMENT;
    const std::string &k = e->keys[rumor];
    *len = (uint32_t)k.size();
    if (!out || cap < k.size()) return GS_ERR_SERIALISATION;
    std::memcpy(out, k.data(), k.size());
    return GS_OK;
}

}

namespace {

gs_status append_frame(int pull, const std::string &msg, uint8_t counter, uint8_t *out, uint32_t cap,
                       uint32_t *len) {
    uint32_t need = 0;
    gs_rpc_encode(pull, nullptr, 0, 0, nullptr, 0, &need);
    need += (uint32_t)msg.size();
    const uint32_t at = *len;
    *len += 4 + need;
    if (!out || *len > cap) return GS_ERR_SERIALISATION;
    for (int i = 0; i < 4; ++i) out[at + i] = (uint8_t)(need >> (8 * i));
    uint32_t w = 0;
    return gs_rpc_encode(pull, reinterpret_cast<const uint8_t *>(msg.data()), (uint32_t)msg.size(), counter,
                         out + at + 4, need, &w);
}

gs_status ext_ready(const gs_engine *e) {
    if (e->round == 0 || !e->deliver_pending) return GS_ERR_INVALID_ARGUMENT;
    if (e->shard && e->pulled_round != e->round) return GS_ERR_INVALID_ARGUMENT;
    return GS_OK;
}

bool ext_ids(const gs_engine *e, uint32_t node, uint32_t peer) {
    if (e->shard) return node >= e->sp.lo && node - e->sp.lo < e->sp.m && peer >= e->n_global;
    return node < e->g.n && peer >= e->g.n;
}

uint32_t slice_own_ext_limit(const gs_engine *e) { return std::min<uint32_t>(200u, 32u * e->g.rpad); }
uint32_t slice_ext_limit(const gs_engine *e) { return e->ext_limit ? e->ext_limit : slice_own_ext_limit(e); }
// ... 300 lines not shown
        auto it = e->key_rumor.find(std::string(reinterpret_cast<const char *>(msg + off), mlen));
        if (it == e->key_rumor.end()) return GS_ERR_INVALID_ARGUMENT;
        rumor = it->second;
    }
    if (e->faults.churn && gs::offline_of(e->seed, e->epoch, e->round, gnode, e->faults.churn)) return GS_OK;
    st = set_device(e);
    if (st != GS_OK) return st;
    const bool fresh = !e->ext_peers.count({node, peer});
    if (fresh && !pull && e->slice && e->ext_fp[node] >= slice_ext_limit(e)) return GS_ERR_DEVICE_LIMIT;
    const bool new_copy = !empty && !e->ext_copy_peers.count({node, rumor, peer});
    if (new_copy) {
        auto c = e->ext_copies.find({node, rumor});
        if (c != e->ext_copies.end() && c->second >= gs::kExtCopiesMax) return GS_ERR_DEVICE_LIMIT;
    }
    const bool is_new = e->ext_peers.insert({node, peer}).second;
    if (is_new && !pull) {
        std::vector<uint16_t> codes;
        st = observe_node(e, node, codes);
        if (st != GS_OK) return st;
        gs_status res = GS_OK;
        for (uint32_t r : e->key_order) {
            const uint32_t tag = codes[r] >> 14;
            if (tag == 1 || tag == 2) {
                const uint8_t c = tag == 1 ? (uint8_t)((codes[r] >> 7) & 0x7Fu) : 255;
                if (append_frame(1, e->keys[r], c, out, cap, out_len) != GS_OK) res = GS_ERR_SERIALISATION;
                ++*out_count;
            }
        }
        if (*out_count == 0) {
            if (append_frame(1, std::string(), 0, out, cap, out_len) != GS_OK) res = GS_ERR_SERIALISATION;
            *out_count = 1;
        }
        if (res != GS_OK) {
            e->ext_peers.erase({node, peer});
            return res;
        }
        ++e->ext_fp[node];
    }
    uint32_t info = (pull ? 0u : gs::kExtPush) | (is_new ? gs::kExtNew : 0u);
    if (empty) {
        info |= gs::kExtEmpty;
    } else {
        e->started = true;
        info |= rumor | ((uint32_t)counter << 12) | gs::kExtRec;
        for (auto &x : e->ext)
            if (x.node == node && x.peer == peer && !(x.info & gs::kExtEmpty) && (x.info & 0xFFFu) == rumor)
                x.info &= ~gs::kExtRec;
    }
    if (new_copy) {
        e->ext_copy_peers.insert({node, rumor, peer});
        ++e->ext_copies[{node, rumor}];
    }
    e->ext.push_back({node, (uint32_t)e->ext.size(), info, peer});
    e->ext_uploaded = (uint32_t)-1;
    e->obs_valid = false;
    return GS_OK;
}

double gs_round_kernel_bytes(const gs_engine *e) {
    if (!e) return 0.0;
    const double n = e->g.n, rp = e->g.rpad;
    if (e->dlv && e->shard) return n * (2.0 * rp + 56.0);
    if (e->dlv) return n * (2.0 * rp + (e->dlv_pack ? 38.0 : 42.0));
    return n * (2.75 * rp + 68.0);
}

const char *gs_round_kernel_name(const gs_engine *e) {
    if (!e) return "";
    if (e->shard && e->dlv) {
        if (e->g.rpad < 16) return "round_kernel_dlv4<1,u32,4,SHARD>";
        return e->dlv_pack == 2 ? "round_kernel_dlv4<1,u64,4,SHARD>"
                                : (e->dlv_pack == 3 ? "round_kernel_dlv4<1,u32,1,SHARD>" : "round_kernel_dlv4<1,u32,2,SHARD>");
    }
    if (e->shard) return e->g.small ? "round_kernel<true,1,SHARD>" : "round_kernel<false,1,SHARD>";
    if (e->seq) return e->g.small ? "round_kernel<true,1,SEQ>" : "round_kernel<false,1,SEQ>";
    if (e->dlv) {
        if (e->dlv_pack == 0) return "round_kernel<true,1,DLV> (one node per lane)";
        if (e->g.rpad < 16) return "round_kernel_dlv4<1,u32,4>";
        return e->dlv_pack == 2 ? "round_kernel_dlv4<1,u64,4>"
                                : (e->dlv_pack == 3 ? "round_kernel_dlv4<1,u32,1>" : "round_kernel_dlv4<1,u32,2>");
    }
    if (e->filt && e->w32 && (e->g.small ? e->g.rpad == 32 : e->g.logr <= 8))
        return "round_kernel_w32<1> (32-bit lanes, live-filtered gathers)";
    if (e->filt) return e->g.small ? "round_kernel<true,1> (live-filtered gathers)"
                                   : "round_kernel<false,1> (live-filtered gathers)";
    return e->g.small ? "round_kernel<true,1>" : "round_kernel<false,1>";
}

gs_status gs_round_traffic(gs_engine *e, double *bytes_per_launch, uint32_t *launches) {
    if (!e || !bytes_per_launch || !launches) return GS_ERR_INVALID_ARGUMENT;
    const double dense = gs_round_kernel_bytes(e);
    if (e->filt) {
        gs_status st = set_device(e);
        if (st != GS_OK) return st;
        *launches = e->filt_launches;
        if (e->filt_launches == 0) {
            *bytes_per_launch = dense;
            return GS_OK;
        }
        u64 rows = 0;
        GS_HIP(hipStreamSynchronize(e->stream));
        GS_HIP(hipMemcpy(&rows, e->acct, sizeof(u64), hipMemcpyDeviceToHost));
        const double n = e->g.n, rp = e->g.rpad;
        *bytes_per_launch = n * (68.0 + 3.0 / 8.0 + 2.0 * rp) + 3.0 * rp / 8.0 * (double)rows / e->filt_launches;
        return GS_OK;
    }
    *bytes_per_launch = dense;
    *launches = 0;
    return GS_OK;
}

}
```

safe_gossip_amd/csrc/gs_inlist.hip:

```cpp
#include <cstdlib>

#include "gs_kernels.h"
#include "gs_device.h"

namespace gs {

namespace {

#ifndef GS_INL_BINLOG
#define GS_INL_BINLOG 14
#endif
constexpr uint32_t kBinLog = GS_INL_BINLOG;
constexpr uint32_t kBin = 1u << kBinLog;
constexpr uint32_t kBinCap = kBin + kBin / 4;
#ifndef GS_INL_CHUNK
#define GS_INL_CHUNK 8192
#endif
constexpr uint32_t kChunk = GS_INL_CHUNK;
constexpr uint32_t kInlThreads = 1024;
static_assert(kChunk % kInlThreads == 0, "inl_bin: whole sources per thread");
constexpr uint32_t kChunkSmall = 2048;
static_assert(kChunkSmall % kInlThreads == 0, "inl_bin: whole sources per thread");
constexpr uint32_t kBinnedMaxBins = 1u << (27 - kBinLog);
#ifndef GS_SORT_OWN_TAILS
#define GS_SORT_OWN_TAILS 1
#endif
#ifndef GS_DLV_OWN_TAILS
#define GS_DLV_OWN_TAILS 1
#endif
constexpr uint32_t kFlagLimit = 2u;

GS_DEV uint32_t target_of(const InListArgs &a, uint32_t x) {
    return target_word(a.seed, a.epoch, a.round, x, a.p.n, a.f);
}

template <bool SH>
GS_DEV void dlv_source(const InListArgs &a, uint32_t x, uint32_t &t, uint32_t &code, uint32_t &src) {
    if constexpr (SH) {
        t = kTgDead;
        code = 0u;
        src = x;
        const uint32_t per = a.sr.P * a.sr.capP, ks = x / per, kr = x - ks * per, kh = kr / a.sr.capP;
        if (x < a.nkeys && (ks != a.self_rank || kr - kh * a.sr.capP < a.self_cnt[kh])) {
            const uint2 r = reinterpret_cast<const uint2 *>(a.rowsA)[shard_key_slot(a.sr, x)];
            if (r.y != 0xFFFFFFFFu) {
                t = r.y & ~kRowMutual;
                code = r.x;
                src = x | (r.y & kRowMutual);
            }
        }
    } else {
        t = target_of(a, x);
        a.tg[x] = t;
        code = a.PC[x];
        src = x;
    }
}

GS_DEV void shard_pull_store(const InListArgs &a, uint32_t key, uint32_t v) {
    const uint32_t b = shard_key_bslot(a.sr, key);
    const bool own = key / (a.sr.P * a.sr.capP) == a.self_rank;
    if (own) a.pullB_self[b] = v;
    if (!own || a.sr.G > 1) a.pullB[b] = v;
}

constexpr uint32_t kLiveTag = 1u << 31;
GS_DEV uint32_t emit_target(const InListArgs &a, uint32_t y, const uint32_t *lst, uint32_t k,
                            uint32_t first, bool yc = false, bool yl = true) {
    InRec r;
    if (k > kMaxIn) {
        atomicOr(&a.flags[2], kFlagLimit);
        k = kMaxIn;
    }
    r.kf = (first << kFirstShift) | k;
    const bool filt = a.lvm != nullptr;
    uint32_t lv = 0;
    if (filt) {
#pragma unroll
        for (uint32_t i = 0; i < kInline; ++i)
            if (i < k && (lst[i] & kLiveTag)) lv |= 1u << i;
    }
#pragma unroll
    for (uint32_t i = 0; i < kInline; ++i) r.s[i] = i < k ? (lst[i] & kIdMask) : 0u;
    if (filt) r.kf |= (~lv & 7u) << kInSkipShift;
    a.IN8[y] = r;
    uint32_t rows = filt ? (uint32_t)__popc(lv) + (k > kInline ? k - kInline : 0u) : 0u;
    bool any_live = false;
    for (uint32_t j = 1; j < k; ++j) {
        const uint32_t prev = j - 1u;
        any_live |= filt && (lst[prev] & kLiveTag) != 0;
        const bool zneed = any_live && !yc;
        if (filt && !zneed) continue;
        if (filt)
            rows += (uint32_t)__popc(lv & ((1u << min(j, kSibInline)) - 1u)) +
                    (j > kSibInline ? j - kSibInline : 0u) + (yl ? 0u : 1u);
        SibRec sr;
        sr.tag = ((a.serial & kSerialMask) << 8) | j | (zneed ? kSibZNeed : 0u) |
                 (filt ? ((~lv & 3u) << kSibSkipShift) : 0u);
#pragma unroll
        for (uint32_t i = 0; i < kSibInline; ++i) sr.e[i] = i < j ? (lst[i] & kIdMask) : 0u;
        if (filt && !((lv >> 2) & 1u)) sr.e[2] |= kSkipBit;
        a.SIB8[lst[j] & kIdMask] = sr;
    }
    return rows;
}

template <uint32_t INL = kInline>
GS_DEV uint32_t tail_len(uint32_t k) { return k > INL ? min(k, kMaxIn) - INL : 0u; }

template <uint32_t NT>
GS_DEV uint32_t reserve_tails(const InListArgs &a, uint32_t mine, uint32_t *tailcnt, uint32_t *lds_scan) {
    __shared__ uint32_t blk_first;
    uint32_t total;
    const uint32_t off = block_exclusive_scan_t<NT>(mine, lds_scan, total);
    if (threadIdx.x == 0) {
        uint32_t f = total ? atomicAdd(tailcnt, total) : 0u;
        if (f + total > a.p.tailcap) {
            atomicOr(&a.flags[2], kFlagLimit);
            f = kNone;
        }
        blk_first = f;
    }
    __syncthreads();
    return blk_first == kNone ? kNone : blk_first + off;
}

GS_DEV uint32_t emit_tail(const InListArgs &a, const uint32_t *lst, uint32_t k, uint32_t &cur) {
    const uint32_t m = tail_len<>(k);
    if (m == 0 || cur == kNone) return 0u;
    const uint32_t first = cur;
    for (uint32_t j = 0; j < m; ++j) a.src[first + j] = lst[kInline + j] & kIdMask;
    cur += m;
    return first;
}

template <uint32_t CHUNK>
__global__ __launch_bounds__(kInlThreads) void inl_bin(InListArgs a) {
    constexpr uint32_t kChunk = CHUNK;
    constexpr uint32_t kBinPer = kChunk / kInlThreads;
    extern __shared__ __attribute__((aligned(16))) uint32_t sh[];
    const CsrPlan &p = a.p;
    uint32_t *stage = sh;
    uint16_t *stage_lt = reinterpret_cast<uint16_t *>(sh + kChunk);
    const uint32_t np = p.nb << p.sub, plog = kBinLog - p.sub, pcap = kBinCap >> p.sub;
    uint32_t *fill = a.scratch + p.fill_off;
    uint32_t *cnt = sh + kChunk + kChunk / 2;
    uint16_t *cnt16 = reinterpret_cast<uint16_t *>(cnt);
    uint16_t *off = reinterpret_cast<uint16_t *>(cnt + (np + 1) / 2);
    uint16_t *res = off + np;
    uint16_t *stage_b = res + np;
    __shared__ uint32_t lds_scan[kInlThreads / 64];
    __shared__ uint32_t zrows;
    if (blockIdx.x == 0 && threadIdx.x == 0) a.scratch[p.nb] = 0u;
    if (threadIdx.x == 0) zrows = 0u;
    for (uint32_t i = threadIdx.x; i < (np + 1) / 2; i += kInlThreads) cnt[i] = 0u;
    __syncthreads();
    const uint32_t lo = blockIdx.x * kChunk;
    const uint32_t hi = min(p.n, lo + kChunk);
    uint32_t tq[kBinPer];
#pragma unroll
    for (uint32_t q = 0; q < kBinPer; ++q) {
        const uint32_t x = lo + threadIdx.x + q * kInlThreads;
        tq[q] = kTgDead;
        if (x < hi) {
            tq[q] = target_of(a, x);
            a.tg[x] = tq[q];
            if (!(tq[q] & kTgDead)) {
// ... 1139 lines not shown
```

safe_gossip_amd/csrc/gs_kernels.h:

```cpp
#pragma once
#include "gs_common.h"

namespace gs {

struct ShardRows {
    uint32_t G, P, W, capP, idrows, rw, rwb, codes, chunk, n;
};

struct RoundArgs {
    const u64 *Scur;
    u64 *Snext;
    const InRec *IN8;
    const SibRec *SIB8;
    const DlvRec *DR;
    const uint32_t *dtail;
    const uint32_t *pull;
    uint32_t *pc_out;
    uint16_t *kn_out;
    uint32_t dlv_tlog, dlv_tper;
    uint32_t *zero_buf;
    uint32_t zero_words;
    u64 *zero_rows;
    const uint4 *IN;
    const uint32_t *IN2;
    const uint32_t *src;
    const uint32_t *tg;
    const uint32_t *tg_next;
    uint32_t serial;
    uint32_t *st32;
    uint32_t st16;
    const u64 *st64;
    u64 obs_rounds;
    const u64 *inj_key;
    const u64 *inj_mask;
    uint32_t n_inj;
    uint32_t *flags;
    uint32_t *live;
    u64 *obs_known;
    u64 *obs_stats;
    uint16_t *obs_state;
    uint16_t *obs_rec;
    uint32_t *obs_psize;
    u64 *obs_digest;
    u64 *obs_dpart;
    uint32_t dp_lo, dp_words;
    const u64 *recvA;
    const u64 *recvB;
    u64 *sendA;
    u64 *recvA_next;
    const uint32_t *spos_cur;
    const uint32_t *spos_next;
    ShardRows sp;
    Faults f;
    u64 *pend;
    uint32_t *offc;
    uint32_t node_lo;
    const u64 *Wb;
    const uint8_t *sinfo;
    const u64 *ext;
    uint32_t n_ext;
    uint32_t blk_off, blk_count, obs_only;
    const uint32_t *blk_list, *obs_list;
    uint32_t n_obs;
    u64 *acct;
    const u64 *zlm;
    u64 *lvm, *cpm;
    const u64 *rows_cnt;
    uint8_t *emin;
    const uint8_t *eadd;
    uint32_t w32;
    uint32_t *zero_buf2;
    uint32_t zero_words2;
    uint32_t dlv_pack;
    Geometry g;
    uint64_t seed;
    uint32_t epoch;
    uint32_t round_new;
    uint32_t cmax, maxc, maxr;
};
constexpr uint32_t kExtPush = 1u << 20, kExtNew = 1u << 21, kExtRec = 1u << 22, kExtEmpty = 1u << 23;
inline u64 node_map_words(uint32_t n) { return ((u64)n + 63u) / 64u + 1u; }
__host__ __device__ inline bool map_test(const u64 *m, uint32_t i) { return ((m[i >> 6] >> (i & 63u)) & 1ull) != 0; }

hipError_t launch_round(const RoundArgs &a, int mode, hipStream_t s);
hipError_t launch_round_dlv4(const RoundArgs &a, int mode, hipStream_t s);
constexpr uint32_t kLiveSlots = 64, kLiveStride = 32;
__device__ __forceinline__ void mark_any_live(uint32_t *live, uint32_t round_new, uint32_t bid, bool blk_live) {
    if (bid == 0 && threadIdx.x < kLiveSlots)
        __hip_atomic_store(&live[(((round_new + 1u) & 1u) * kLiveSlots + threadIdx.x) * kLiveStride], 0u,
                           __ATOMIC_RELAXED, __HIP_MEMORY_SCOPE_AGENT);
    if (threadIdx.x == 0 && blk_live)
        __hip_atomic_store(&live[((round_new & 1u) * kLiveSlots + (bid & (kLiveSlots - 1u))) * kLiveStride], 1u,
                           __ATOMIC_RELAXED, __HIP_MEMORY_SCOPE_AGENT);
}
constexpr uint32_t kTileNodes = 64;
inline uint64_t tile_padded(uint64_t n) { return (n + kTileNodes - 1) / kTileNodes * kTileNodes; }
bool w32_eligible(const RoundArgs &a, int mode);
hipError_t launch_round_w32(const RoundArgs &a, int mode, hipStream_t s);

struct CsrPlan {
    uint32_t n;
    uint32_t binned;
    uint32_t bin;
    uint32_t logbin;
    uint32_t nb;
    uint32_t ba;
    uint32_t chunk;
    uint32_t tailcap;
    uint32_t dlv;
    uint32_t sub;
    uint32_t fill_off;
};
CsrPlan csr_plan(uint32_t n);
CsrPlan dlv_plan(uint32_t n);
struct InListSizes {
    size_t src_words, region_words, scratch_words;
};
InListSizes inlist_sizes(const CsrPlan &p);
void inlist_zero_range(const CsrPlan &p, size_t *first, size_t *words);
void inlist_cfill_range(const CsrPlan &p, size_t *first, size_t *words);

struct InListArgs {
    CsrPlan p;
    uint32_t *tg;
    uint32_t dlv;
    const u64 *S;
    const uint32_t *PC;
    const uint16_t *KN;
    uint32_t prezeroed;
    Geometry g;
    DlvRec *DR;
    uint32_t *dtail;
    uint32_t *pull;
    InRec *IN8;
    SibRec *SIB8;
    uint32_t *src;
    uint32_t *region;
    uint32_t *scratch;
    uint32_t *flags;
    uint32_t serial;
    uint64_t seed;
    uint32_t epoch, round;
    Faults f;
    const u64 *lvm, *cpm;
    u64 *zl;
    u64 *rows;
    const uint32_t *rowsA;
    uint32_t *pullB;
    ShardRows sr;
    uint32_t nkeys, ntargets;
    uint32_t self_rank;
    const uint32_t *self_cnt;
    uint32_t *pullB_self;
};
hipError_t launch_build_inlists(const InListArgs &a, hipStream_t s);
void dlv_tail_parts(const CsrPlan &p, uint32_t *log, uint32_t *per);
hipError_t launch_stats_fold(uint32_t *st32, u64 *st64, uint32_t n, uint32_t st16, hipStream_t s);
hipError_t launch_slice_apply(uint32_t *st32, const uint8_t *emin, uint32_t n, uint32_t st16, hipStream_t s);

struct SeqArgs {
    const u64 *S;
    const InRec *IN8;
    const SibRec *SIB8;
    const uint32_t *src;
    const uint32_t *tg;
    uint32_t serial;
    uint8_t *sinfo;
    u64 *Wb;
// ... 124 lines not shown
```

safe_gossip_amd/csrc/gs_kernels.hip:

```cpp
#include "gs_kernels.h"
#include "gs_device.h"
#include "gs_recv.h"

namespace gs {

#ifndef GS_RK_SMALL_BLK
#define GS_RK_SMALL_BLK 64u
#endif
constexpr uint32_t kRkSmallBlk = GS_RK_SMALL_BLK;
static_assert(kRkSmallBlk == 64u || kRkSmallBlk == 128u, "a thread's stage step must cover whole nodes at W <= 16");

#ifndef GS_RK_MINW
#define GS_RK_MINW 1
#endif
#ifndef GS_RK_MINW_SMALL
#define GS_RK_MINW_SMALL 1
#endif
#ifndef GS_RK_ZSKIP
#define GS_RK_ZSKIP 1
#endif
#ifndef GS_RK_ZSKIP_BLK
#define GS_RK_ZSKIP_BLK 0
#endif

#ifndef GS_RK_TAILPRE
#define GS_RK_TAILPRE 1
#endif

GS_DEV Cls decode16(uint32_t code) {
    const u64 b0 = code & 0xFFFFu, b1 = code >> 16;
    return Cls{b0 & b1, b0 & ~b1, b1 & ~b0};
}

template <bool SMALL, int MODE, bool SHARD, bool SEQ, bool DLV, uint32_t BLK = 256u, bool EXT = false>
__global__ __launch_bounds__(BLK, BLK == 256u ? GS_RK_MINW : GS_RK_MINW_SMALL) void round_kernel(RoundArgs a) {
    constexpr bool DELIVER = (MODE == 1 || MODE == 2);
    static_assert(!EXT || DELIVER, "external RPCs are applied with the round's deliveries");
    constexpr bool TRANSITION = (MODE == 0 || MODE == 1);
    const Geometry &g = a.g;
    constexpr uint32_t kBlk = BLK;
    static_assert(BLK == 256u || (!SMALL && !SEQ && !DLV && (MODE == 0 || MODE == 1)),
                  "smaller blocks: gather-path and class-row shard transitions only");
    constexpr uint32_t kBlockWords = kBlk * kPlanes;
    constexpr uint32_t kStageIters = kBlockWords / 2u / kBlk;
    constexpr uint32_t kStageWords = kBlockWords + kBlockWords / 4u;
    if (a.zero_buf || a.zero_rows) zero_for_build(a.zero_buf, a.zero_words, a.zero_rows);
    if (a.zero_buf2) zero_for_build(a.zero_buf2, a.zero_words2, nullptr);
    const uint32_t bid = (!TRANSITION && a.blk_list) ? a.blk_list[blockIdx.x] : blockIdx.x + a.blk_off;
    const u64 seg = (u64)bid * blockDim.x + threadIdx.x;
    const bool valid = seg < g.nseg;
    Lane<SMALL> L;
    L.init(g, valid ? seg : 0);
    const uint32_t x = L.x;
    const u64 *__restrict__ S = a.Scur;

    __shared__ uint32_t blk_any;
    __shared__ uint32_t blk_nz;
    if (threadIdx.x == 0) blk_any = 0;
    if (threadIdx.x == 0) blk_nz = 0;
    __builtin_amdgcn_s_setprio(2);

    __shared__ __attribute__((aligned(16))) u64 stage[kStageWords];
    const uint32_t wlog = SMALL ? 0u : g.logr - 6u;
    const uint32_t pst = SMALL ? 0u : (9u << wlog) + (wlog == 0u ? 1u : 0u);
    auto sidx = [&](uint32_t li) -> uint32_t {
        return SMALL ? li : (li >> (wlog + 3u)) * pst + (li & ((8u << wlog) - 1u));
    };
    const uint32_t s4 = sidx(2u * threadIdx.x), s4d = SMALL ? 2u * kBlk : ((kBlk / 4u) >> wlog) * pst;
    const uint32_t npu_blk = SMALL ? (1u << g.lognpu) : 1u;
    const u64 blk_base = (u64)bid * (kBlockWords / npu_blk);
    const uint32_t blk_v4 = (uint32_t)min((u64)(kBlockWords / npu_blk),
                                          g.units * kPlanes * (SMALL ? 1u : g.W) - blk_base) / 2u;
    static_assert(kStageIters == 4, "stage loads are unrolled by hand");
    const uint4 *src4 = reinterpret_cast<const uint4 *>(S + blk_base);
    const uint4 st0 = src4[min(threadIdx.x, blk_v4 - 1u)];
    const uint4 st1 = src4[min(threadIdx.x + kBlk, blk_v4 - 1u)];
    const uint4 st2 = src4[min(threadIdx.x + 2u * kBlk, blk_v4 - 1u)];
    const uint4 st3 = src4[min(threadIdx.x + 3u * kBlk, blk_v4 - 1u)];

    uint4 stv = {0u, 0u, 0u, 0u};
    if (TRANSITION && valid && (SMALL || L.j == 0)) stv = load_stats(a.st32, a.st16, x);
    uint32_t eadd = 0;
    if (TRANSITION && a.eadd && valid && (SMALL || L.j == 0)) eadd = reinterpret_cast<const uint16_t *>(a.eadd)[x];
    uint4 in = {0, 0, 0, 0};
    InRec in8 = {};
    SibRec sb8 = {};
    uint32_t z = x, zi = 0xFFFFu, k = 0, r = 0;
    uint32_t tgw = 0;
    uint32_t sinf = 0;
    bool seq_inl = false;
    bool seq_dep = false;
    DlvRec dr = {};
    uint32_t dpull = 0;
    const bool filt = !SHARD && !SEQ && !DLV && a.zlm != nullptr;
    u64 zlw = 0;
    uint32_t qskip = 0;
    uint32_t eskip = 0;
    bool zneed = false;
    bool gq[kBatchK], ge[kBatchE], gz = true;
#pragma unroll
    for (uint32_t i = 0; i < kBatchK; ++i) gq[i] = true;
#pragma unroll
    for (uint32_t i = 0; i < kBatchE; ++i) ge[i] = true;
    if (DELIVER) {
        if (DLV) {
            dr = a.DR[x];
            tgw = a.tg[x];
            dpull = a.pull[x];
            z = tgw & kTgMask;
            k = valid ? (dr.mf & 31u) : 0u;
        } else if (SHARD) {
            if (valid) {
                in = a.IN[x];
                zi = in.y >> 16;
                k = in.y & 0xFFFFu;
                if (faults_on(a.f)) tgw = a.tg[x];
            }
        } else {
            in8 = a.IN8[x];
            tgw = a.tg[x];
            z = tgw & kTgMask;
            k = valid ? in8.k() : 0u;
            if (SEQ) sinf = a.sinfo[x];
            sb8 = a.SIB8[x];
            if (filt) zlw = a.zlm[x >> 6];
            const bool sib_ok = valid && (sb8.tag >> 8) == (a.serial & kSerialMask);
            r = sib_ok ? (sb8.tag & kSibRankMask) : 0u;
            if (filt) {
                qskip = in8.kf >> kInSkipShift;
                in8.kf &= kInFlagMask;
                eskip = ((sb8.tag >> kSibSkipShift) & 3u) | ((sb8.e[2] >> 31) << 2);
                sb8.e[2] &= kIdMask;
                zneed = sib_ok && (sb8.tag & kSibZNeed) != 0;
            }
            if (SEQ) {
                seq_inl = valid && (sinf & kSeqGot) && (sinf & kSeqLevelMask) == kSeqInline;
                seq_dep = seq_inl && (sinf & kSeqDep);
                if (!seq_inl) r = 0;
            }
        }
    }

    Cls q[kBatchK], e[kBatchE], qz = {0, 0, 0}, wz = {0, 0, 0};
    uint32_t tail0 = 0;
#pragma unroll
    for (uint32_t i = 0; i < kBatchK; ++i) q[i] = {0, 0, 0};
#pragma unroll
    for (uint32_t i = 0; i < kBatchE; ++i) e[i] = {0, 0, 0};
    if (DELIVER) {
        if (DLV) {
        } else if (SHARD) {
            if (valid) {
                static_assert(kBatchK == 3, "shard rows: three batched pushers");
                const uint32_t e2 = a.IN2[x];
                const uint32_t sp = a.spos_cur[x];
                q[0] = L.load_push_row(a.recvA, in.z);
                q[1] = L.load_push_row(a.recvA, in.w);
                q[2] = L.load_push_row(a.recvA, e2);
                gz = !(tgw & kTgNoPull) && sp != 0xFFFFFFFFu;
                if (gz) {
                    qz.c = a.recvB[L.row_index(sp, 2, 0)];
                    qz.a0 = a.recvB[L.row_index(sp, 2, 1)];
                    qz.a1 = 0;
                }
            }
        } else if (filt) {
            if (!SEQ && k > kInline) tail0 = a.src[in8.first()];
#pragma unroll
            for (uint32_t i = 0; i < kBatchK; ++i) {
                gq[i] = i < k && !((qskip >> i) & 1u);
                if (gq[i]) q[i] = L.load_cls(S, in8.s[i]);
            }
            gz = valid && !(tgw & kTgNoPull) && (((zlw >> (x & 63u)) & 1ull) != 0 || zneed);
            if (gz) qz = L.load_cls(S, z);
#pragma unroll
            for (uint32_t i = 0; i < kBatchE; ++i) {
                ge[i] = i < r && !((eskip >> i) & 1u);
                if (ge[i]) e[i] = L.load_cls(S, sb8.e[i]);
            }
        } else {
            if (!SEQ && k > kInline) tail0 = a.src[in8.first()];
#pragma unroll
            for (uint32_t i = 0; i < kBatchK; ++i) q[i] = L.load_cls(S, i < k ? in8.s[i] : x);
            if (SEQ && !seq_inl) {
                if (valid && (sinf & kSeqGot)) {
                    const u64 wi = ((u64)x * 2u) * g.W + L.j;
                    qz.c = a.Wb[wi];
                    qz.a0 = a.Wb[wi + g.W];
                }
            } else {
                qz = L.load_cls(S, z);
                if (SEQ && seq_dep) {
                    const u64 wi = ((u64)z * 2u) * g.W + L.j;
                    const u64 b0 = a.Wb[wi], b1 = a.Wb[wi + g.W];
                    wz = Cls{b0 & b1, b0 & ~b1, b1 & ~b0};
                }
            }
            if (!SEQ || seq_inl) {
#pragma unroll
                for (uint32_t i = 0; i < kBatchE; ++i) e[i] = L.load_cls(S, i < r ? sb8.e[i] : x);
            }
        }
    }
    Cls t0 = {0, 0, 0};
    if (GS_RK_TAILPRE && DELIVER && !SEQ && !DLV && !SHARD && k > kInline) t0 = L.load_cls(S, tail0);
    static_assert(kBatchE < kSibInline, "sibling #kBatchE is inline");
    Cls s2 = {0, 0, 0};
    if (GS_RK_TAILPRE && DELIVER && !SEQ && !DLV && !SHARD && r > kBatchE && !(tgw & kTgNoPull) &&
        (!filt || zneed) && !((eskip >> kBatchE) & 1u))
        s2 = L.load_cls(S, pick_sib(sb8.e, kBatchE));
    __builtin_amdgcn_s_setprio(0);
    {
        *reinterpret_cast<uint4 *>(&stage[s4]) = st0;
        *reinterpret_cast<uint4 *>(&stage[s4 + s4d]) = st1;
        *reinterpret_cast<uint4 *>(&stage[s4 + 2u * s4d]) = st2;
        *reinterpret_cast<uint4 *>(&stage[s4 + 3u * s4d]) = st3;
    }
    __syncthreads();
    u64 P[kPlanes];
    const uint32_t sb0 = sidx((uint32_t)(L.plane_index(0) - blk_base));
#pragma unroll
    for (int p = 0; p < kPlanes; ++p) {
        const u64 v = valid ? stage[sb0 + ((uint32_t)p << wlog)] : 0ull;
        P[p] = SMALL ? ((v >> L.sh) & L.m) : v;
    }


    const u64 isC = P[0], a0 = P[1], a1 = P[2];
    const u64 A = ~isC & ~a0 & ~a1 & L.m;
    const u64 B = ~isC & (a0 | a1);
    const u64 C = isC & ~(a0 & a1);
    const u64 D = isC & a0 & a1;
    const u64 liveX = B | C;

    const bool off_t = DELIVER && (tgw & kTgOff);
    const bool pulled = !(tgw & kTgNoPull);
    using RecvT = Recv<!TRANSITION, u64, EXT ? kVoteBitsExt : kVoteBits>;
    RecvT rv;
    rv.init(A, B, B & a0 & ~a1);
    uint32_t psize = 0;
    uint32_t ext_new = 0, ext_full = 0, ext_empty = 0, ext_recv = 0;
    bool seq_gx = false, seq_skip = false;
    uint32_t seq_px = 0, seq_jz = kNone;
    if (DELIVER && valid && k > 30u) atomicOr(&a.flags[2], 1u);
    if (DELIVER && valid) {
        bool zin = false;
        u64 pv2, pvB, pCl;
        if (DLV) {
            static_assert(kDlvInline == 2, "inline pushers are read by hand");
            const uint32_t dzi = (dr.mf >> 5) & 31u;
            const uint32_t dfirst = (x >> a.dlv_tlog) * a.dlv_tper + (dr.mf >> kDlvFirstShift);
            zin = dzi != kDlvNoZ;
            for (uint32_t i = 0; i < k; ++i) {
                const uint32_t code = i == 0 ? dr.c[0] : (i == 1 ? dr.c[1] : a.dtail[dfirst + i - kDlvInline]);
                rv.push(decode16(code), i, k, !(pulled && i == dzi));
            }
            const u64 b0 = dpull & 0xFFFFu, b1 = dpull >> 16;
            pv2 = b1 & ~b0;
            pvB = b0 ^ b1;
            pCl = b0 & b1;
            if (!pulled) pv2 = pvB = pCl = 0;
        } else if (SHARD) {
            zin = zi != 0xFFFFu;
            const uint32_t zs = pulled ? zi : 0xFFFFu;
#pragma unroll
            for (uint32_t i = 0; i < kBatchK; ++i)
                if (i < k) rv.push(q[i], i, k, zs != i);
            for (uint32_t i = kBatchK; i < k; ++i) {
                rv.push(L.load_push_row(a.recvA, a.src[in.x + i]), i, k, zs != i);
            }
            pv2 = qz.a0 & ~qz.c;
            pvB = qz.c ^ qz.a0;
            pCl = qz.c & qz.a0;
        } else if (SEQ) {
            const bool gx = (sinf & kSeqGot) != 0;
            uint32_t px = 0, jz = kNone;
            for (uint32_t i = 0; i < k; ++i) {
                const uint32_t s = i < kInline ? pick_inline(in8.s, i) : a.src[in8.first() + (i - kInline)];
                px += s < x ? 1u : 0u;
                if (s == z) jz = i;
            }
            zin = jz != kNone;
            if (seq_inl) {
                const u64 zB = ~qz.c & (qz.a0 | qz.a1);
                const u64 zC = qz.c & ~(qz.a0 & qz.a1);
                u64 pnot = ~qz.c & ~qz.a0 & ~qz.a1 & L.m, pB = 0, pC = 0;
                bool wdone = !seq_dep;
                auto put_w = [&](uint32_t s) {
                    if (!wdone && s > z) {
                        sibling(wz, pnot, pB, pC);
                        wdone = true;
                    }
                };
#pragma unroll
                for (uint32_t i = 0; i < kBatchE; ++i)
                    if (i < r) {
                        put_w(sb8.e[i]);
                        sibling(e[i], pnot, pB, pC);
                    }
                if (r > kBatchE && (pnot || !wdone)) {
                    for (uint32_t i = kBatchE; i < min(r, kSibInline); ++i) {
                        const uint32_t s = pick_sib(sb8.e, i);
                        put_w(s);
                        sibling(L.load_cls(S, s), pnot, pB, pC);
                    }
                    if (r > kSibInline && (pnot || !wdone)) {
                        const InRec zin8 = a.IN8[z];
                        for (uint32_t i = kSibInline; i < r && (pnot || !wdone); ++i) {
                            const uint32_t s = i < kInline ? pick_inline(zin8.s, i)
                                                           : a.src[zin8.first() + (i - kInline)];
                            put_w(s);
                            sibling(L.load_cls(S, s), pnot, pB, pC);
                        }
                    }
                }
                if (!wdone) sibling(wz, pnot, pB, pC);
                const u64 pcl = zC | pC;
                const u64 b0 = ((zB & qz.a0 & ~qz.a1) | pB | pcl) & L.m;
                const u64 b1 = ((zB & qz.a1 & ~qz.a0) | pcl) & L.m;
                qz = Cls{b0, b1, 0};
            }
            const bool skip = gx && zin && z > x;
            const uint32_t sk = skip ? 1u : 0u;
            u64 precm = ~0ull;
            if (zin && z > x) {
                Cls qj = L.load_cls(S, z);
                const u64 vCj = qj.c & ~(qj.a0 & qj.a1);
                precm = ~((~qj.c & (qj.a0 | qj.a1)) | vCj);
            }
            pv2 = qz.a0 & ~qz.c;
            pvB = qz.c ^ qz.a0;
            pCl = qz.c & qz.a0;
            bool pdone = !gx;
            for (uint32_t i = 0; i < k; ++i) {
                if (!pdone && i == px) {
                    rv.absorb(pvB, pv2, pCl, k - px - sk, px, precm);
                    pdone = true;
                }
                Cls qi;
                if (i < kBatchK) {
                    qi = q[0];
#pragma unroll
                    for (uint32_t b = 1; b < kBatchK; ++b) qi = (i == b) ? q[b] : qi;
                } else {
                    qi = L.load_cls(S, a.src[in8.first() + (i - kInline)]);
                }
                const uint32_t rafter = (k - 1u - i) - ((skip && jz > i) ? 1u : 0u);
                rv.absorb_cls(qi, rafter, i + ((gx && i >= px) ? 1u : 0u), !(i == jz && gx && z < x));
            }
            if (!pdone) rv.absorb(pvB, pv2, pCl, 0u, px, precm);
            seq_gx = gx;
            seq_px = px;
            seq_jz = jz;
            seq_skip = skip;
            pv2 = pvB = pCl = 0;
        } else {
#pragma unroll
            for (uint32_t i = 0; i < kBatchK; ++i) {
                if (i < k) {
                    zin |= in8.s[i] == z;
                    if (!filt || gq[i]) rv.push(q[i], i, k, !(pulled && in8.s[i] == z));
                }
            }
            for (uint32_t i = kBatchK; i < k; ++i) {
                const uint32_t s = i < kInline ? pick_inline(in8.s, i)
                                               : (i == kInline ? tail0 : a.src[in8.first() + (i - kInline)]);
                zin |= s == z;
                rv.push((GS_RK_TAILPRE && i == kInline) ? t0 : L.load_cls(S, s), i, k, !(pulled && s == z));
            }
            const u64 zB = ~qz.c & (qz.a0 | qz.a1);
            const u64 zC = qz.c & ~(qz.a0 & qz.a1);
            u64 pnot = ~qz.c & ~qz.a0 & ~qz.a1 & L.m, pB = 0, pC = 0;
#pragma unroll
            for (uint32_t i = 0; i < kBatchE; ++i)
                if (i < r && (!filt || ge[i])) sibling(e[i], pnot, pB, pC);
            if (r > kBatchE && pnot && pulled && (!filt || zneed)) {
                auto sib_row = [&](uint32_t s, bool skip) -> Cls {
                    if (skip) return Cls{0, 0, 0};
                    return L.load_cls(S, s);
                };
                for (uint32_t i = kBatchE; i < min(r, kSibInline); ++i) {
                    const bool sk = ((eskip >> i) & 1u) != 0;
                    Cls row;
                    if (GS_RK_TAILPRE && i == kBatchE) {
                        row = s2;
                    } else {
                        row = sib_row(pick_sib(sb8.e, i), sk);
                    }
                    sibling(row, pnot, pB, pC);
                }
                if (r > kSibInline && pnot) {
                    InRec zin8 = a.IN8[z];
                    if (filt) zin8.kf &= kInFlagMask;
                    for (uint32_t i = kSibInline; i < r && pnot; ++i) {
                        const uint32_t s = i < kInline ? pick_inline(zin8.s, i)
                                                       : a.src[zin8.first() + (i - kInline)];
                        sibling(sib_row(s, false), pnot, pB, pC);
                    }
                }
            }
            pv2 = zB & qz.a1 & ~qz.a0;
            pvB = zB | pB;
            pCl = zC | pC;
            if (!pulled) pv2 = pvB = pCl = 0;
        }
        const u64 pl = pvB | pCl;
        {
            const u64 newc = rv.notyet & pl;
            rv.record(rv.recB & pl, pvB, pv2, pCl);
            rv.create(newc, pCl);
        }
        rv.recv += popc(pl);
        if (a.n_ext) {
            uint32_t lo = 0, hi = a.n_ext;
            const u64 key = (u64)x << 32;
            while (lo < hi) {
                const uint32_t mid = (lo + hi) >> 1;
                if (a.ext[mid] < key) lo = mid + 1; else hi = mid;
            }
            for (uint32_t i = lo; i < a.n_ext && (uint32_t)(a.ext[i] >> 32) == x; ++i) {
                const uint32_t info = (uint32_t)a.ext[i];
                if (info & kExtNew) ++ext_new;
                if ((info & kExtPush) && (info & kExtNew)) {
                    uint32_t cnt = popc((B | C | rv.crB | rv.crC) & L.m);
                    if (!SMALL) cnt = group_sum(cnt, g.W);
                    if (cnt) ext_full += cnt; else ++ext_empty;
                }
                if (info & kExtEmpty) continue;
                ++ext_recv;
                const uint32_t r = info & 0xFFFu, c = (info >> 12) & 0xFFu;
                if ((SMALL ? 0u : (r >> 6)) != L.j) continue;
                const u64 bit = 1ull << (SMALL ? r : (r & 63u));
                const u64 vC = c >= a.cmax ? bit : 0ull;
                const u64 vB = (c >= 1u && c < a.cmax) ? bit : 0ull;
                const u64 v2 = (c == 2u && c < a.cmax) ? bit : 0ull;
                const u64 newc = rv.notyet & bit;
                rv.record(rv.recB & bit & ((info & kExtRec) ? ~0ull : 0ull), vB, v2, vC);
                rv.create(newc, vC);
            }
        }
        const bool gets = SEQ ? seq_gx : pulled;
        psize = k + ((gets && !zin) ? 1u : 0u) + ext_new;
    }
    const u64 crB = rv.crB, crC = rv.crC, anyC = rv.anyC;

    uint32_t lc = popc(liveX);
    uint32_t part_cw = rv.part_cw, recv = rv.recv, first_create = rv.first_create;
    if (DELIVER && !SMALL) {
        lc = group_sum(lc, g.W);
        part_cw = group_sum(part_cw, g.W);
        recv = group_sum(recv, g.W);
        first_create = group_min(first_create, g.W);
    }
    uint32_t d_full_sent = 0, d_empty_pull = 0, d_recv = 0;
    if (DELIVER && SEQ) {
        const uint32_t nresp = k - (seq_skip ? 1u : 0u);
        d_full_sent = nresp * lc + part_cw;
        if (nresp > 0 && lc == 0) {
            if (first_create == kNone) {
                d_empty_pull = nresp;
            } else {
                uint32_t c = (!seq_gx || first_create < seq_px) ? first_create + 1u : first_create;
                c = min(c, k);
                if (seq_skip && seq_jz + 1u <= first_create) c -= 1u;
                d_empty_pull = c;
            }
        }
// ... 79 lines not shown
        }
        if (a.obs_digest) {
            const uint32_t jw = SMALL ? 0u : L.j;
            u64 dg = 64u * jw < g.R ? digest_word(jw, L.m, B, C, D, crB, crC, a0, a1, &P[3], anyC, rv.c1, rv.c2) : 0ull;
            if (!SMALL)
                for (uint32_t o = 1; o < g.W; o <<= 1) dg += __shfl_xor(dg, (int)o, 64);
            if (leader) a.obs_digest[x] += dg;
        }
        if (a.obs_state || a.obs_rec) {
            const uint32_t nb = SMALL ? g.rpad : 64u;
            for (uint32_t b = 0; b < nb; ++b) {
                const uint32_t rr = SMALL ? b : L.j * 64u + b;
                if (rr >= g.R) break;
                const u64 bit = 1ull << b;
                uint32_t bf = 0;
#pragma unroll
                for (int i = 0; i < 5; ++i) bf |= (uint32_t)((P[3 + i] >> b) & 1u) << i;
                const uint32_t af = (uint32_t)((a0 >> b) & 1u) | ((uint32_t)((a1 >> b) & 1u) << 1);
                uint16_t code = 0;
                if (crB & bit) code = (uint16_t)((1u << 14) | (1u << 7));
                else if (crC & bit) code = (uint16_t)(2u << 14);
                else if (B & bit) code = (uint16_t)((1u << 14) | (af << 7) | bf);
                else if (C & bit) code = (uint16_t)((2u << 14) | (af << 7) | bf);
                else if (D & bit) code = (uint16_t)(3u << 14);
                if (a.obs_state) a.obs_state[(u64)x * g.R + rr] = code;
                if (a.obs_rec) {
                    uint16_t rvv = 0;
                    if ((B | crB) & bit) {
                        uint32_t v1 = 0, v2 = 0;
#pragma unroll
                        for (int i = 0; i < RecvT::kNB; ++i) {
                            v1 |= (uint32_t)((rv.c1[i] >> b) & 1u) << i;
                            v2 |= (uint32_t)((rv.c2[i] >> b) & 1u) << i;
                        }
                        rvv = (uint16_t)((((anyC >> b) & 1u) << 15) | (v2 << 7) | v1);
                    }
                    a.obs_rec[(u64)x * g.R + rr] = rvv;
                }
            }
        }
        return;
    }

    u64 N[kPlanes];
    u64 Bn = 0, Cn = 0;
    bool on_next = true;
    {
        u64 inj = 0;
        if (a.n_inj && valid) inj = find_injection(a, SMALL ? (u64)x : seg) & L.m;
        on_next = !(a.f.churn && valid && offline_of(a.seed, a.epoch, a.round_new, a.node_lo + x, a.f.churn));
        const u64 pidx = ((u64)x * 2u) * g.W + L.j;
        const bool pending = off_t && valid;
        const u64 pb = pending ? a.pend[pidx] : 0ull, pa = pending ? a.pend[pidx + g.W] : 0ull;
        NextOut o;
        next_round_seg(P, rv, inj, psize, pending, pb, pa, on_next, a.cmax, a.maxc, a.maxr, o);
#pragma unroll
        for (int p = 0; p < kPlanes; ++p) N[p] = o.N[p];
        Bn = o.Bn;
        Cn = o.Cn;
        if (!on_next) {
            a.pend[pidx] = o.bump;
            a.pend[pidx + g.W] = o.anyC;
        }
    }

    if (DLV && valid) {
        const u64 vC = N[0] & ~(N[1] & N[2]), vB = ~N[0] & (N[1] | N[2]);
        const u64 b0 = ((vB & N[1] & ~N[2]) | vC) & L.m, b1 = ((vB & N[2] & ~N[1]) | vC) & L.m;
        a.pc_out[x] = (uint32_t)b0 | ((uint32_t)b1 << 16);
        if (a.kn_out) a.kn_out[x] = (uint16_t)((N[0] | N[1] | N[2]) & L.m);
    }

    if (TRANSITION && a.lvm) {
        u64 lvw, aw;
        if (a.f.churn == 0u) {
            lvw = Bn | Cn;
            aw = ~(N[0] | Bn) & L.m;
        } else {
            lvw = ((N[0] & ~(N[1] & N[2])) | (~N[0] & (N[1] | N[2]))) & L.m;
            aw = ~N[0] & ~N[1] & ~N[2] & L.m;
        }
        const u64 bl = __ballot(valid && lvw != 0);
        const u64 bc = __ballot(valid && aw == 0);
        const uint32_t lane = threadIdx.x & 63u;
        const u64 seg0 = seg - lane;
        if (lane == 0 && seg0 < g.nseg) {
            if (SMALL) {
                a.lvm[seg0 >> 6] = bl;
                a.cpm[seg0 >> 6] = bc;
            } else {
                const uint32_t lw = g.logr - 6u;
                const u64 cl = compress_stride(group_or_bits(bl, lw), lw);
                const u64 cc = compress_stride(group_and_bits(bc, lw), lw);
                uint8_t *ml = reinterpret_cast<uint8_t *>(a.lvm), *mc = reinterpret_cast<uint8_t *>(a.cpm);
                const u64 byte0 = (seg0 >> lw) >> 3;
                if (lw == 0u) {
                    *reinterpret_cast<u64 *>(ml + byte0) = cl;
                    *reinterpret_cast<u64 *>(mc + byte0) = cc;
                } else if (lw == 1u) {
                    *reinterpret_cast<uint32_t *>(ml + byte0) = (uint32_t)cl;
                    *reinterpret_cast<uint32_t *>(mc + byte0) = (uint32_t)cc;
                } else if (lw == 2u) {
                    *reinterpret_cast<uint16_t *>(ml + byte0) = (uint16_t)cl;
                    *reinterpret_cast<uint16_t *>(mc + byte0) = (uint16_t)cc;
                } else {
                    ml[byte0] = (uint8_t)cl;
                    mc[byte0] = (uint8_t)cc;
                }
            }
        }
        if (MODE == 1 && a.acct && a.rows_cnt && bid == 0 && threadIdx.x == 0) atomicAdd(a.acct, *a.rows_cnt);
    }

    uint32_t live_new = (valid && on_next) ? popc(Bn | Cn) : 0u;
    if (!SMALL) live_new = group_sum(live_new, g.W);
    if (__ballot(live_new != 0u) != 0ull && (threadIdx.x & 63u) == 0u) blk_any = 1u;
    constexpr bool kZBlk = GS_RK_ZSKIP_BLK && TRANSITION && kBlk != 64u;
    const u64 nz_mask = SMALL ? L.m : ~0ull;
    if (kZBlk && __ballot(valid && ((N[0] | N[1] | N[2]) & nz_mask) != 0ull) != 0ull && (threadIdx.x & 63u) == 0u)
        blk_nz = 1u;
    __syncthreads();
    const bool blk_live = blk_any != 0u;
    __builtin_amdgcn_s_setprio(1);
    const bool zskip = kZBlk ? blk_nz == 0u
                             : GS_RK_ZSKIP && kBlk == 64u && __ballot(valid && (N[0] | N[1] | N[2]) != 0ull) == 0ull;
    if (zskip) {
    } else if (SMALL) {
        const uint32_t npu = 1u << g.lognpu;
#pragma unroll
        for (int p = 0; p < kPlanes; ++p) {
            u64 v = valid ? ((N[p] & L.m) << L.sh) : 0ull;
            for (uint32_t o = 1; o < npu; o <<= 1) v |= __shfl_xor(v, (int)o, 64);
            if (valid && (x & (npu - 1u)) == 0) stage[sidx((uint32_t)(L.plane_index(p) - blk_base))] = v;
        }
    } else if (valid) {
#pragma unroll
        for (int p = 0; p < kPlanes; ++p) stage[sb0 + ((uint32_t)p << wlog)] = N[p];
    }
    if (!zskip) __syncthreads();
    if (!zskip) {
        uint4 *dst4 = reinterpret_cast<uint4 *>(a.Snext + blk_base);
        for (uint32_t i = threadIdx.x, si = s4; i < blk_v4; i += blockDim.x, si += s4d)
            nt_store4(*reinterpret_cast<const uint4 *>(&stage[si]), &dst4[i]);
    }
    if (SHARD) {
        const uint32_t sp = valid ? a.spos_next[x] : 0xFFFFFFFFu;
        const u64 vC = N[0] & ~(N[1] & N[2]), vB = ~N[0] & (N[1] | N[2]);
        const u64 c0 = ((vB & N[1] & ~N[2]) | vC) & L.m;
        const u64 c1 = ((vB & N[2] & ~N[1]) | vC) & L.m;
        if (sp != 0xFFFFFFFFu) {
            a.sendA[L.row_index(sp, 2, 0)] = c0;
            a.sendA[L.row_index(sp, 2, 1)] = c1;
        }
    }

    mark_any_live(a.live, a.round_new, bid, blk_live);
    if (leader) {
        uint4 v = stv;
        if (a.st16 && (ext_full | ext_empty | ext_recv)) {
            u64 *s64 = const_cast<u64 *>(a.st64) + (u64)x * 4u;
            if (!a.emin) {
                s64[0] += ext_empty;
                d_empty_pull -= ext_empty;
            }
            s64[2] += ext_full;
            s64[3] += ext_recv;
            d_full_sent -= ext_full;
            d_recv -= ext_recv;
        }
        const uint32_t d_empty_push = (on_next && live_new == 0u) ? 1u : 0u;
        if (a.emin) {
            reinterpret_cast<uint16_t *>(a.emin)[x] = (uint16_t)(min(d_empty_pull, 255u) | (d_empty_push << 8));
            v.x += eadd & 0xFFu;
            v.y += eadd >> 8;
        } else {
            v.x += d_empty_pull;
            v.y += d_empty_push;
        }
        v.z += live_new + d_full_sent;
        v.w += d_recv;
        store_stats(a.st32, a.st16, x, v);
        if (!on_next) atomicAdd(&a.offc[x], 1u);
    }
}

template <bool SMALL, bool SHARD, bool SEQ, bool DLV = false>
static hipError_t launch_mode(const RoundArgs &a, int mode, hipStream_t s) {
    const bool ext = a.n_ext > 0 && (mode == 1 || mode == 2);
    if constexpr (!SMALL && !SEQ && !DLV) {
        if ((mode == 0 || mode == 1) && a.g.W <= 16u) {
            if (a.blk_list) return hipErrorInvalidValue;
            constexpr u64 f = 256u / kRkSmallBlk;
            const u64 nblk = (a.g.nseg + kRkSmallBlk - 1) / kRkSmallBlk;
            const u64 b0 = std::min<u64>((u64)a.blk_off * f, nblk);
            const u64 b1 = a.blk_count ? std::min<u64>(((u64)a.blk_off + a.blk_count) * f, nblk) : nblk;
            if (b1 <= b0) return hipSuccess;
            RoundArgs b = a;
            b.blk_off = (uint32_t)b0;
            if (mode == 0)
                hipLaunchKernelGGL((round_kernel<false, 0, SHARD, false, false, kRkSmallBlk>), dim3((uint32_t)(b1 - b0)),
                                   dim3(kRkSmallBlk), 0, s, b);
            else if (ext)
                hipLaunchKernelGGL((round_kernel<false, 1, SHARD, false, false, kRkSmallBlk, true>),
                                   dim3((uint32_t)(b1 - b0)), dim3(kRkSmallBlk), 0, s, b);
            else
                hipLaunchKernelGGL((round_kernel<false, 1, SHARD, false, false, kRkSmallBlk>), dim3((uint32_t)(b1 - b0)),
                                   dim3(kRkSmallBlk), 0, s, b);
            return hipGetLastError();
        }
    }
    const uint32_t block = 256;
    const u64 grid = a.blk_count ? a.blk_count : (a.g.nseg + block - 1) / block;
    if (grid == 0) return hipSuccess;
    if (a.blk_list && (mode == 0 || mode == 1)) return hipErrorInvalidValue;
    switch (mode) {
    case 0: hipLaunchKernelGGL((round_kernel<SMALL, 0, SHARD, SEQ, DLV>), dim3((uint32_t)grid), dim3(block), 0, s, a); break;
    case 1:
        if (ext) hipLaunchKernelGGL((round_kernel<SMALL, 1, SHARD, SEQ, DLV, 256u, true>), dim3((uint32_t)grid), dim3(block), 0, s, a);
        else hipLaunchKernelGGL((round_kernel<SMALL, 1, SHARD, SEQ, DLV>), dim3((uint32_t)grid), dim3(block), 0, s, a);
        break;
    case 2:
        if (ext) hipLaunchKernelGGL((round_kernel<SMALL, 2, SHARD, SEQ, DLV, 256u, true>), dim3((uint32_t)grid), dim3(block), 0, s, a);
        else hipLaunchKernelGGL((round_kernel<SMALL, 2, SHARD, SEQ, DLV>), dim3((uint32_t)grid), dim3(block), 0, s, a);
        break;
    default: hipLaunchKernelGGL((round_kernel<SMALL, 3, SHARD, SEQ, DLV>), dim3((uint32_t)grid), dim3(block), 0, s, a); break;
    }
    return hipGetLastError();
}

hipError_t launch_round(const RoundArgs &a, int mode, hipStream_t s) {
    if (a.recvA) {
        if (a.sp.codes) return (mode == 0 || mode == 1) ? launch_round_dlv4(a, mode, s) : hipErrorInvalidValue;
        return a.g.small ? launch_mode<true, true, false>(a, mode, s) : launch_mode<false, true, false>(a, mode, s);
    }
    if (a.Wb)
        return a.g.small ? launch_mode<true, false, true>(a, mode, s) : launch_mode<false, false, true>(a, mode, s);
    if (a.DR) {
        if (!a.g.small || a.g.rpad > 16) return hipErrorInvalidValue;
        if (a.dlv_pack && (mode == 0 || mode == 1)) return launch_round_dlv4(a, mode, s);
        return launch_mode<true, false, false, true>(a, mode, s);
    }
    if (w32_eligible(a, mode)) return launch_round_w32(a, mode, s);
    return a.g.small ? launch_mode<true, false, false>(a, mode, s) : launch_mode<false, false, false>(a, mode, s);
}

__global__ __launch_bounds__(256) void slice_apply(uint32_t *st32, const uint8_t *__restrict__ emin, uint32_t n,
                                                   uint32_t st16) {
    const uint32_t x = blockIdx.x * blockDim.x + threadIdx.x;
    if (x >= n) return;
    uint4 v = load_stats(st32, st16, x);
    v.x += emin[2u * (u64)x];
    v.y += emin[2u * (u64)x + 1u];
    store_stats(st32, st16, x, v);
}

hipError_t launch_slice_apply(uint32_t *st32, const uint8_t *emin, uint32_t n, uint32_t st16, hipStream_t s) {
    if (n == 0) return hipSuccess;
    hipLaunchKernelGGL(slice_apply, dim3((n + 255u) / 256u), dim3(256), 0, s, st32, emin, n, st16);
    return hipGetLastError();
}

__global__ __launch_bounds__(256) void stats_fold(uint32_t *st32, u64 *st64, u64 words, uint32_t st16) {
    const u64 i = (u64)blockIdx.x * blockDim.x + threadIdx.x;
    if (i >= words) return;
    if (st16) {
        uint16_t *s16 = reinterpret_cast<uint16_t *>(st32);
        st64[i] += s16[i];
        s16[i] = 0;
    } else {
        st64[i] += st32[i];
        st32[i] = 0u;
    }
}

hipError_t launch_stats_fold(uint32_t *st32, u64 *st64, uint32_t n, uint32_t st16, hipStream_t s) {
    const u64 words = (u64)n * 4;
    if (words == 0) return hipSuccess;
    hipLaunchKernelGGL(stats_fold, dim3((uint32_t)((words + 255) / 256)), dim3(256), 0, s, st32, st64,
                       words, st16);
    return hipGetLastError();
}

__global__ __launch_bounds__(256) void known_reduce(const u64 *__restrict__ known, uint32_t n,
                                                    uint32_t KW, uint32_t min_known, u64 *partials) {
    __shared__ u64 s_tot[256], s_cmp[256];
    u64 tot = 0, cmp = 0;
    for (u64 x = (u64)blockIdx.x * blockDim.x + threadIdx.x; x < n; x += (u64)gridDim.x * blockDim.x) {
        uint32_t c = 0;
        for (uint32_t w = 0; w < KW; ++w) c += popc(known[x * KW + w]);
        tot += c;
        cmp += (c >= min_known) ? 1u : 0u;
    }
    s_tot[threadIdx.x] = tot;
    s_cmp[threadIdx.x] = cmp;
    __syncthreads();
    for (uint32_t o = 128; o > 0; o >>= 1) {
        if (threadIdx.x < o) {
            s_tot[threadIdx.x] += s_tot[threadIdx.x + o];
            s_cmp[threadIdx.x] += s_cmp[threadIdx.x + o];
        }
        __syncthreads();
    }
    if (threadIdx.x == 0) {
        partials[2 * blockIdx.x] = s_tot[0];
        partials[2 * blockIdx.x + 1] = s_cmp[0];
    }
}

hipError_t launch_known_reduce(const u64 *known, uint32_t n, uint32_t KW, uint32_t min_known,
                               u64 *partials, uint32_t blocks, hipStream_t s) {
    hipLaunchKernelGGL(known_reduce, dim3(blocks), dim3(256), 0, s, known, n, KW, min_known, partials);
    return hipGetLastError();
}

__global__ __launch_bounds__(256) void known_popc(const u64 *__restrict__ known, uint32_t n, uint32_t KW,
                                                  uint32_t *counts) {
    const u64 x = (u64)blockIdx.x * blockDim.x + threadIdx.x;
    if (x >= n) return;
    uint32_t c = 0;
    for (uint32_t w = 0; w < KW; ++w) c += popc(known[x * KW + w]);
    counts[x] = c;
}

hipError_t launch_known_popc(const u64 *known, uint32_t n, uint32_t KW, uint32_t *counts, hipStream_t s) {
    if (n == 0) return hipSuccess;
    hipLaunchKernelGGL(known_popc, dim3((n + 255) / 256), dim3(256), 0, s, known, n, KW, counts);
    return hipGetLastError();
}
// ... 72 lines not shown
```

Measured before the change: 1944 billion.

## Add worklist path that runs the full round only on non-trivial waves

Splits the delivering round into a light pre-pass kernel and a persistent worklist kernel. The pre-pass bumps the stats of quiet nodes directly and compacts the waves that still have work into a list; the persistent round kernel then processes only listed waves. A host-side growth estimate, refreshed from a pinned-memory counter, switches back to the dense kernel once the active share passes a threshold. The aim is to avoid reading the full state when few waves are live, at the cost of an extra launch, atomics, the per-wave nonzero marks and the heuristic's risk of choosing the wrong path.

```diff
diff --git a/include/safe_gossip.h b/include/safe_gossip.h
--- a/include/safe_gossip.h
+++ b/include/safe_gossip.h
@@ -98,6 +98,7 @@
 double      gs_round_kernel_bytes(const gs_engine *e);
 const char *gs_round_kernel_name(const gs_engine *e);
 gs_status   gs_round_traffic(gs_engine *e, double *bytes_per_launch, uint32_t *launches);
+gs_status   gs_round_path_info(gs_engine *e, uint32_t out[4]);
 
 gs_status   gs_shard_create(const gs_config *cfg, uint32_t rank, uint32_t world, gs_engine **out);
 gs_status   gs_shard_create_parts(const gs_config *cfg, uint32_t rank, uint32_t world, uint32_t parts,
diff --git a/safe_gossip_amd/__init__.py b/safe_gossip_amd/__init__.py
--- a/safe_gossip_amd/__init__.py
+++ b/safe_gossip_amd/__init__.py
@@ -120,6 +120,7 @@
     "gs_round_kernel_bytes": (ctypes.c_double, [_P]),
     "gs_round_kernel_name": (ctypes.c_char_p, [_P]),
     "gs_round_traffic": (ctypes.c_int, [_P, ctypes.POINTER(ctypes.c_double), _U32P]),
+    "gs_round_path_info": (ctypes.c_int, [_P, _U32P]),
     "gs_peer": (ctypes.c_uint32, [ctypes.c_uint64, ctypes.c_uint32, ctypes.c_uint32,
                                   ctypes.c_uint32, ctypes.c_uint32]),
     "gs_origin": (ctypes.c_uint32, [ctypes.c_uint64, ctypes.c_uint32, ctypes.c_uint32,
@@ -677,6 +678,11 @@
         _check(self._lib.gs_round_traffic(self._h, ctypes.byref(b), ctypes.byref(m)))
         return float(b.value), int(m.value)
 
+    def round_path_info(self):
+        out = (ctypes.c_uint32 * 4)()
+        _check(self._lib.gs_round_path_info(self._h, out))
+        return int(out[0]), int(out[1]), int(out[2]) | (int(out[3]) << 32)
+
 
 class Gossiper:
 
diff --git a/safe_gossip_amd/csrc/gs_common.h b/safe_gossip_amd/csrc/gs_common.h
--- a/safe_gossip_amd/csrc/gs_common.h
+++ b/safe_gossip_amd/csrc/gs_common.h
@@ -136,6 +136,7 @@
 };
 constexpr uint32_t kInSkipShift = 28;
 constexpr uint32_t kInFlagMask = (1u << kInSkipShift) - 1u;
+constexpr uint32_t kInTailLive = 1u << 31;
 constexpr uint32_t kSibSkipShift = 5;
 constexpr uint32_t kSkipBit = 1u << 31;
 constexpr uint32_t kIdMask = kSkipBit - 1u;
diff --git a/safe_gossip_amd/csrc/gs_device.h b/safe_gossip_amd/csrc/gs_device.h
--- a/safe_gossip_amd/csrc/gs_device.h
+++ b/safe_gossip_amd/csrc/gs_device.h
@@ -7,6 +7,11 @@
 
 GS_DEV uint32_t popc(u64 v) { return (uint32_t)__popcll(v); }
 
+GS_DEV void zero_for_build(uint32_t *buf, uint32_t words, u64 *one, uint32_t bdim) {
+    const uint32_t gt = blockIdx.x * bdim + threadIdx.x;
+    for (uint32_t i = gt; i < words; i += gridDim.x * bdim) buf[i] = 0u;
+    if (one && gt == 0u) *one = 0ull;
+}
 GS_DEV void zero_for_build(uint32_t *buf, uint32_t words, u64 *one) {
     const uint32_t gt = blockIdx.x * blockDim.x + threadIdx.x;
     for (uint32_t i = gt; i < words; i += gridDim.x * blockDim.x) buf[i] = 0u;
diff --git a/safe_gossip_amd/csrc/gs_engine.cpp b/safe_gossip_amd/csrc/gs_engine.cpp
--- a/safe_gossip_amd/csrc/gs_engine.cpp
+++ b/safe_gossip_amd/csrc/gs_engine.cpp
@@ -55,6 +55,20 @@
     uint32_t dlv_pack = 1;
     bool w32 = false;
     u64 *acct = nullptr;
+    bool wl_ok = false;
+    int wl_mode = -1;
+    bool wl_dense = false;
+    bool ra_wl = false;
+    uint8_t *wnz = nullptr;
+    uint32_t *wl_list = nullptr, *wl_cnt = nullptr;
+    uint32_t wl_par = 0;
+    u64 *wl_total = nullptr;
+    u64 *wl_host = nullptr;
+    uint32_t wl_gen = 0;
+    double wl_est = 0.0;
+    uint32_t wl_grid = 0;
+    uint32_t path_wl = 0, path_dense = 0;
+    uint32_t acct_wl = 0;
     uint32_t *pc = nullptr;
     uint16_t *kn = nullptr;
     hipStream_t cstream = nullptr;
@@ -130,6 +144,8 @@
 
 constexpr uint32_t kReduceBlocks = 1024;
 constexpr uint32_t kTimingSlots = 4096;
+constexpr double kWlDenseShare = 0.375;
+constexpr double kWlGrowth = 3.5;
 
 void report_hip(hipError_t err, const char *what, int line) {
     static const bool on = [] {
@@ -188,12 +204,13 @@
     }
     if (e->ev_main) (void)hipEventDestroy(e->ev_main);
     if (e->cstream) (void)hipStreamDestroy(e->cstream);
-    void *bufs[] = {e->lvm, e->cpm, e->rows_dev, e->acct, e->pc, e->kn, e->Wb, e->sinfo, e->seqw, e->pend, e->offc, e->S[0], e->S[1], e->flags, e->live, e->st32, e->st64, e->inj_key, e->inj_mask, e->obs_known, e->obs_stats,
+    void *bufs[] = {e->wnz, e->wl_list, e->wl_cnt, e->wl_total, e->lvm, e->cpm, e->rows_dev, e->acct, e->pc, e->kn, e->Wb, e->sinfo, e->seqw, e->pend, e->offc, e->S[0], e->S[1], e->flags, e->live, e->st32, e->st64, e->inj_key, e->inj_mask, e->obs_known, e->obs_stats,
                     e->partials, e->obs_state, e->obs_rec, e->obs_psize, e->obs_digest, e->obs_pend, e->ext_dev,
                     e->node_state, e->batch_lists, e->batch_codes};
     for (void *b : bufs)
         if (b) (void)hipFree(b);
     if (e->inj_host) (void)hipHostFree(e->inj_host);
+    if (e->wl_host) (void)hipHostFree(e->wl_host);
     for (hipEvent_t ev : e->tev) (void)hipEventDestroy(ev);
     if (e->stream) (void)hipStreamDestroy(e->stream);
     delete e;
@@ -216,6 +233,14 @@
         gs::inlist_cfill_range(e->plan, &first, &words);
         for (auto &c : e->csr)
             if (words && c.scratch) GS_HIP(hipMemsetAsync(c.scratch + first, 0, words * sizeof(uint32_t), e->stream));
+    }
+    if (e->wl_ok) {
+        GS_HIP(hipMemsetAsync(e->wnz, 0, (size_t)gs::wave_count(g), e->stream));
+        GS_HIP(hipMemsetAsync(e->wl_total, 0, sizeof(u64), e->stream));
+        ++e->wl_gen;
+        e->wl_dense = false;
+        e->wl_est = 0.0;
+        e->path_wl = e->path_dense = 0;
     }
     e->cur = 0;
     e->round = 0;
@@ -311,6 +336,12 @@
             a.zlm = cs.zl;
             a.lvm = e->lvm;
             a.cpm = e->cpm;
+        }
+        if (e->wl_ok) {
+            a.wnz = e->wnz;
+            a.wl_list = e->wl_list;
+            a.wl_cnt = e->wl_cnt;
+            a.wl_total = e->wl_total;
         }
     }
     a.st32 = e->st32;
@@ -704,6 +735,11 @@
         const bool off = v && *v == '0';
         e->filt = !off && !e->shard && !e->seq && !e->dlv && e->plan.binned && (g.small || g.W <= 8);
     }
+    {
+        const char *v = std::getenv("SAFE_GOSSIP_AMD_WORKLIST");
+        e->wl_mode = (v && *v) ? (*v != '0' ? 1 : 0) : -1;
+        e->wl_ok = e->filt && !g.small && g.W <= 8 && !e->w32 && !e->slice && !gs::faults_on(e->faults);
+    }
     e->st16 = e->dlv;
     e->fold_every = (uint32_t)std::max<uint64_t>(1, (e->st16 ? 0xFFFFull : 0xFFFFFFFFull) / (32ull * g.rpad + 32) / 2);
     bool ok;
@@ -759,7 +795,17 @@
         ok = dalloc(&e->lvm, gs::node_map_words(n)) == hipSuccess &&
              dalloc(&e->cpm, gs::node_map_words(n)) == hipSuccess &&
              dalloc(&e->rows_dev, 2) == hipSuccess &&
-             dalloc(&e->acct, 1) == hipSuccess && hipMemsetAsync(e->acct, 0, sizeof(u64), e->stream) == hipSuccess;
+             dalloc(&e->acct, 2) == hipSuccess && hipMemsetAsync(e->acct, 0, 2 * sizeof(u64), e->stream) == hipSuccess;
+    if (ok && e->wl_ok) {
+        const size_t waves = (size_t)gs::wave_count(g);
+        ok = dalloc(&e->wnz, waves) == hipSuccess && dalloc(&e->wl_list, waves) == hipSuccess &&
+             dalloc(&e->wl_cnt, 2) == hipSuccess && dalloc(&e->wl_total, 1) == hipSuccess &&
+             hipMemsetAsync(e->wl_cnt, 0, 2 * sizeof(uint32_t), e->stream) == hipSuccess &&
+             hipMemsetAsync(e->wnz, 0, waves, e->stream) == hipSuccess &&
+             hipHostMalloc((void **)&e->wl_host, sizeof(u64), 0) == hipSuccess &&
+             gs::worklist_resident_blocks(e->device, &e->wl_grid) == hipSuccess && e->wl_grid > 0;
+        if (ok) *e->wl_host = 0;
+    }
     if (ok && e->seq)
         ok = dalloc(&e->Wb, (size_t)n * 2 * g.W) == hipSuccess && dalloc(&e->sinfo, n) == hipSuccess &&
              dalloc(&e->seqw, (size_t)gs::seq_blocks(n) * gs::kSeqLists + gs::kSeqLists + n) == hipSuccess;
@@ -1033,6 +1079,33 @@
         a.rows_cnt = e->rows_dev + (R0 & 1u);
         e->filt_launches++;
     }
+    e->ra_wl = false;
+    const uint32_t wl_tag = (e->wl_gen << 16) | (R0 & 0xFFFFu);
+    if (e->wl_ok) {
+        const double waves = (double)gs::wave_count(e->g);
+        double est = e->wl_est + n_inj;
+        e->wl_est = std::min(waves, kWlGrowth * est);
+        if (e->wl_mode < 0 && !e->wl_dense) {
+            const u64 v = __atomic_load_n(e->wl_host, __ATOMIC_RELAXED);
+            const uint32_t tag = (uint32_t)(v >> 32), lag = (R0 - tag) & 0xFFFFu;
+            if ((tag >> 16) == (e->wl_gen & 0xFFFFu) && lag >= 1u && lag < 64u)
+                est = (double)(uint32_t)v * std::pow(kWlGrowth, (double)lag) + n_inj;
+            if (est > kWlDenseShare * waves) e->wl_dense = true;
+        }
+        if (e->wl_mode != 0 && gs::worklist_eligible(a, e->deliver_pending ? 1 : 0))
+            e->ra_wl = e->wl_mode > 0 || !e->wl_dense;
+    }
+    if (e->ra_wl) {
+        a.wl_par = e->wl_par;
+        e->wl_par ^= 1u;
+        a.wl_host = e->wl_host;
+        a.wl_tag = wl_tag;
+        if (a.acct) {
+            a.wl_acct = e->acct + 1;
+            e->acct_wl++;
+        }
+    }
+    if (e->wl_ok && e->deliver_pending) ++(e->ra_wl ? e->path_wl : e->path_dense);
     if (e->shard) {
         GS_HIP(hipStreamWaitEvent(e->stream, e->ev_plan[(R0 + 1) % 3], 0));
         if (e->deliver_pending && !e->dlv) GS_HIP(hipStreamWaitEvent(e->stream, e->ev_edges[R0 % 2], 0));
@@ -1092,7 +1165,8 @@
         e->lt1 = t1;
     }
     if (t0) GS_HIP(hipEventRecord(t0, e->stream));
-    GS_HIP(gs::launch_round(a, e->ra_mode, e->stream));
+    if (e->ra_wl) GS_HIP(gs::launch_round_worklist(a, e->wl_grid, e->stream));
+    else GS_HIP(gs::launch_round(a, e->ra_mode, e->stream));
     if (t1) GS_HIP(hipEventRecord(t1, e->stream));
     return GS_OK;
 }
@@ -1417,7 +1491,7 @@
     e->tcount = 0;
     if (e->timing && e->filt) {
         (void)hipSetDevice(e->device);
-        if (hipMemsetAsync(e->acct, 0, sizeof(u64), e->stream) == hipSuccess) e->filt_launches = 0;
+        if (hipMemsetAsync(e->acct, 0, 2 * sizeof(u64), e->stream) == hipSuccess) e->filt_launches = e->acct_wl = 0;
     }
 }
 
@@ -1884,6 +1958,10 @@
     }
     if (e->filt && e->w32 && (e->g.small ? e->g.rpad == 32 : e->g.logr <= 8))
         return "round_kernel_w32<1> (32-bit lanes, live-filtered gathers)";
+    if (e->filt && e->wl_ok && e->wl_mode != 0)
+        return e->wl_mode > 0 ? "round_kernel<false,1> (live-filtered gathers; round_light + worklist of non-trivial waves)"
+                              : "round_kernel<false,1> (live-filtered gathers; round_light + worklist of non-trivial waves "
+                                "while an estimated 3/8 of the waves or fewer)";
     if (e->filt) return e->g.small ? "round_kernel<true,1> (live-filtered gathers)"
                                    : "round_kernel<false,1> (live-filtered gathers)";
     return e->g.small ? "round_kernel<true,1>" : "round_kernel<false,1>";
@@ -1900,11 +1978,16 @@
             *bytes_per_launch = dense;
             return GS_OK;
         }
-        u64 rows = 0;
+        u64 acct[2] = {0, 0};
         GS_HIP(hipStreamSynchronize(e->stream));
-        GS_HIP(hipMemcpy(&rows, e->acct, sizeof(u64), hipMemcpyDeviceToHost));
-        const double n = e->g.n, rp = e->g.rpad;
-        *bytes_per_launch = n * (68.0 + 3.0 / 8.0 + 2.0 * rp) + 3.0 * rp / 8.0 * (double)rows / e->filt_launches;
+        GS_HIP(hipMemcpy(acct, e->acct, sizeof(acct), hipMemcpyDeviceToHost));
+        const double n = e->g.n, rp = e->g.rpad, per_node = 68.0 + 3.0 / 8.0 + 2.0 * rp;
+        const double waves = (double)gs::wave_count(e->g), wl = e->acct_wl, full = e->filt_launches - e->acct_wl;
+        const double listed_nodes = std::min((double)acct[1] * (64.0 / e->g.W), wl * n);
+        const double total = full * n * per_node + listed_nodes * per_node +
+                             wl * (n * gs::kLightNodeRead + waves) + (wl * n - listed_nodes) * gs::kLightNodeWrite +
+                             3.0 * rp / 8.0 * (double)acct[0];
+        *bytes_per_launch = total / e->filt_launches;
         return GS_OK;
     }
     *bytes_per_launch = dense;
@@ -1912,4 +1995,20 @@
     return GS_OK;
 }
 
-}
+gs_status gs_round_path_info(gs_engine *e, uint32_t out[4]) {
+    if (!e || !out) return GS_ERR_INVALID_ARGUMENT;
+    out[0] = out[1] = out[2] = out[3] = 0;
+    if (!e->wl_ok) return GS_OK;
+    gs_status st = set_device(e);
+    if (st != GS_OK) return st;
+    u64 listed = 0;
+    GS_HIP(hipStreamSynchronize(e->stream));
+    GS_HIP(hipMemcpy(&listed, e->wl_total, sizeof(u64), hipMemcpyDeviceToHost));
+    out[0] = e->path_wl;
+    out[1] = e->path_dense;
+    out[2] = (uint32_t)listed;
+    out[3] = (uint32_t)(listed >> 32);
+    return GS_OK;
+}
+
+}
diff --git a/safe_gossip_amd/csrc/gs_inlist.hip b/safe_gossip_amd/csrc/gs_inlist.hip
--- a/safe_gossip_amd/csrc/gs_inlist.hip
+++ b/safe_gossip_amd/csrc/gs_inlist.hip
@@ -83,6 +83,10 @@
 #pragma unroll
     for (uint32_t i = 0; i < kInline; ++i) r.s[i] = i < k ? (lst[i] & kIdMask) : 0u;
     if (filt) r.kf |= (~lv & 7u) << kInSkipShift;
+    if (filt) {
+        for (uint32_t i = kInline; i < k; ++i)
+            if (lst[i] & kLiveTag) r.kf |= kInTailLive;
+    }
     a.IN8[y] = r;
     uint32_t rows = filt ? (uint32_t)__popc(lv) + (k > kInline ? k - kInline : 0u) : 0u;
     bool any_live = false;
diff --git a/safe_gossip_amd/csrc/gs_kernels.h b/safe_gossip_amd/csrc/gs_kernels.h
--- a/safe_gossip_amd/csrc/gs_kernels.h
+++ b/safe_gossip_amd/csrc/gs_kernels.h
@@ -71,6 +71,12 @@
     uint32_t w32;
     uint32_t *zero_buf2;
     uint32_t zero_words2;
+    uint8_t *wnz;
+    uint32_t *wl_list, *wl_cnt;
+    uint32_t wl_par;
+    u64 *wl_host;
+    u64 wl_tag;
+    u64 *wl_total, *wl_acct;
     uint32_t dlv_pack;
     Geometry g;
     uint64_t seed;
@@ -84,6 +90,11 @@
 
 hipError_t launch_round(const RoundArgs &a, int mode, hipStream_t s);
 hipError_t launch_round_dlv4(const RoundArgs &a, int mode, hipStream_t s);
+bool worklist_eligible(const RoundArgs &a, int mode);
+hipError_t launch_round_worklist(const RoundArgs &a, uint32_t grid, hipStream_t s);
+hipError_t worklist_resident_blocks(int device, uint32_t *blocks);
+inline u64 wave_count(const Geometry &g) { return (g.nseg + 63u) / 64u; }
+constexpr double kLightNodeRead = 48.125, kLightNodeWrite = 16.0;
 constexpr uint32_t kLiveSlots = 64, kLiveStride = 32;
 __device__ __forceinline__ void mark_any_live(uint32_t *live, uint32_t round_new, uint32_t bid, bool blk_live) {
     if (bid == 0 && threadIdx.x < kLiveSlots)
diff --git a/safe_gossip_amd/csrc/gs_kernels.hip b/safe_gossip_amd/csrc/gs_kernels.hip
--- a/safe_gossip_amd/csrc/gs_kernels.hip
+++ b/safe_gossip_amd/csrc/gs_kernels.hip
@@ -19,9 +19,6 @@
 #ifndef GS_RK_ZSKIP
 #define GS_RK_ZSKIP 1
 #endif
-#ifndef GS_RK_ZSKIP_BLK
-#define GS_RK_ZSKIP_BLK 0
-#endif
 
 #ifndef GS_RK_TAILPRE
 #define GS_RK_TAILPRE 1
@@ -32,22 +29,26 @@
     return Cls{b0 & b1, b0 & ~b1, b1 & ~b0};
 }
 
-template <bool SMALL, int MODE, bool SHARD, bool SEQ, bool DLV, uint32_t BLK = 256u, bool EXT = false>
-__global__ __launch_bounds__(BLK, BLK == 256u ? GS_RK_MINW : GS_RK_MINW_SMALL) void round_kernel(RoundArgs a) {
+template <bool SMALL, int MODE, bool SHARD, bool SEQ, bool DLV, uint32_t BLK, bool EXT, bool WL>
+GS_DEV void round_block(const RoundArgs &a, const uint32_t wl_bid) {
     constexpr bool DELIVER = (MODE == 1 || MODE == 2);
     static_assert(!EXT || DELIVER, "external RPCs are applied with the round's deliveries");
     constexpr bool TRANSITION = (MODE == 0 || MODE == 1);
+    constexpr bool kTailPre = GS_RK_TAILPRE && !WL;
     const Geometry &g = a.g;
+    uint32_t tid = threadIdx.x;
+    if constexpr (WL) asm volatile("" : "+v"(tid));
     constexpr uint32_t kBlk = BLK;
     static_assert(BLK == 256u || (!SMALL && !SEQ && !DLV && (MODE == 0 || MODE == 1)),
                   "smaller blocks: gather-path and class-row shard transitions only");
     constexpr uint32_t kBlockWords = kBlk * kPlanes;
     constexpr uint32_t kStageIters = kBlockWords / 2u / kBlk;
     constexpr uint32_t kStageWords = kBlockWords + kBlockWords / 4u;
-    if (a.zero_buf || a.zero_rows) zero_for_build(a.zero_buf, a.zero_words, a.zero_rows);
-    if (a.zero_buf2) zero_for_build(a.zero_buf2, a.zero_words2, nullptr);
-    const uint32_t bid = (!TRANSITION && a.blk_list) ? a.blk_list[blockIdx.x] : blockIdx.x + a.blk_off;
-    const u64 seg = (u64)bid * blockDim.x + threadIdx.x;
+    static_assert(!WL || (MODE == 1 && BLK == 64u && !SHARD && !EXT), "worklist launches: the 2P gather path's one-wave MODE 1");
+    if (!WL && (a.zero_buf || a.zero_rows)) zero_for_build(a.zero_buf, a.zero_words, a.zero_rows, kBlk);
+    if (!WL && a.zero_buf2) zero_for_build(a.zero_buf2, a.zero_words2, nullptr, kBlk);
+    const uint32_t bid = WL ? wl_bid : (!TRANSITION && a.blk_list) ? a.blk_list[blockIdx.x] : blockIdx.x + a.blk_off;
+    const u64 seg = (u64)bid * kBlk + tid;
     const bool valid = seg < g.nseg;
     Lane<SMALL> L;
     L.init(g, valid ? seg : 0);
@@ -55,9 +56,7 @@
     const u64 *__restrict__ S = a.Scur;
 
     __shared__ uint32_t blk_any;
-    __shared__ uint32_t blk_nz;
-    if (threadIdx.x == 0) blk_any = 0;
-    if (threadIdx.x == 0) blk_nz = 0;
+    if (tid == 0) blk_any = 0;
     __builtin_amdgcn_s_setprio(2);
 
     __shared__ __attribute__((aligned(16))) u64 stage[kStageWords];
@@ -66,17 +65,17 @@
     auto sidx = [&](uint32_t li) -> uint32_t {
         return SMALL ? li : (li >> (wlog + 3u)) * pst + (li & ((8u << wlog) - 1u));
     };
-    const uint32_t s4 = sidx(2u * threadIdx.x), s4d = SMALL ? 2u * kBlk : ((kBlk / 4u) >> wlog) * pst;
+    const uint32_t s4 = sidx(2u * tid), s4d = SMALL ? 2u * kBlk : ((kBlk / 4u) >> wlog) * pst;
     const uint32_t npu_blk = SMALL ? (1u << g.lognpu) : 1u;
     const u64 blk_base = (u64)bid * (kBlockWords / npu_blk);
     const uint32_t blk_v4 = (uint32_t)min((u64)(kBlockWords / npu_blk),
                                           g.units * kPlanes * (SMALL ? 1u : g.W) - blk_base) / 2u;
     static_assert(kStageIters == 4, "stage loads are unrolled by hand");
     const uint4 *src4 = reinterpret_cast<const uint4 *>(S + blk_base);
-    const uint4 st0 = src4[min(threadIdx.x, blk_v4 - 1u)];
-    const uint4 st1 = src4[min(threadIdx.x + kBlk, blk_v4 - 1u)];
-    const uint4 st2 = src4[min(threadIdx.x + 2u * kBlk, blk_v4 - 1u)];
-    const uint4 st3 = src4[min(threadIdx.x + 3u * kBlk, blk_v4 - 1u)];
+    const uint4 st0 = src4[min(tid, blk_v4 - 1u)];
+    const uint4 st1 = src4[min(tid + kBlk, blk_v4 - 1u)];
+    const uint4 st2 = src4[min(tid + 2u * kBlk, blk_v4 - 1u)];
+    const uint4 st3 = src4[min(tid + 3u * kBlk, blk_v4 - 1u)];
 
     uint4 stv = {0u, 0u, 0u, 0u};
     if (TRANSITION && valid && (SMALL || L.j == 0)) stv = load_stats(a.st32, a.st16, x);
@@ -203,10 +202,10 @@
         }
     }
     Cls t0 = {0, 0, 0};
-    if (GS_RK_TAILPRE && DELIVER && !SEQ && !DLV && !SHARD && k > kInline) t0 = L.load_cls(S, tail0);
+    if (kTailPre && DELIVER && !SEQ && !DLV && !SHARD && k > kInline) t0 = L.load_cls(S, tail0);
     static_assert(kBatchE < kSibInline, "sibling #kBatchE is inline");
     Cls s2 = {0, 0, 0};
-    if (GS_RK_TAILPRE && DELIVER && !SEQ && !DLV && !SHARD && r > kBatchE && !(tgw & kTgNoPull) &&
+    if (kTailPre && DELIVER && !SEQ && !DLV && !SHARD && r > kBatchE && !(tgw & kTgNoPull) &&
         (!filt || zneed) && !((eskip >> kBatchE) & 1u))
         s2 = L.load_cls(S, pick_sib(sb8.e, kBatchE));
     __builtin_amdgcn_s_setprio(0);
@@ -232,6 +231,7 @@
     const u64 C = isC & ~(a0 & a1);
     const u64 D = isC & a0 & a1;
     const u64 liveX = B | C;
+    const bool wave_was_a = kBlk == 64u && TRANSITION && !SHARD && __ballot(valid && (isC | a0 | a1) != 0ull) == 0ull;
 
     const bool off_t = DELIVER && (tgw & kTgOff);
     const bool pulled = !(tgw & kTgNoPull);
@@ -366,7 +366,7 @@
                 const uint32_t s = i < kInline ? pick_inline(in8.s, i)
                                                : (i == kInline ? tail0 : a.src[in8.first() + (i - kInline)]);
                 zin |= s == z;
-                rv.push((GS_RK_TAILPRE && i == kInline) ? t0 : L.load_cls(S, s), i, k, !(pulled && s == z));
+                rv.push((kTailPre && i == kInline) ? t0 : L.load_cls(S, s), i, k, !(pulled && s == z));
             }
             const u64 zB = ~qz.c & (qz.a0 | qz.a1);
             const u64 zC = qz.c & ~(qz.a0 & qz.a1);
@@ -382,7 +382,7 @@
                 for (uint32_t i = kBatchE; i < min(r, kSibInline); ++i) {
                     const bool sk = ((eskip >> i) & 1u) != 0;
                     Cls row;
-                    if (GS_RK_TAILPRE && i == kBatchE) {
+                    if (kTailPre && i == kBatchE) {
                         row = s2;
                     } else {
                         row = sib_row(pick_sib(sb8.e, i), sk);
@@ -628,7 +628,7 @@
         }
         const u64 bl = __ballot(valid && lvw != 0);
         const u64 bc = __ballot(valid && aw == 0);
-        const uint32_t lane = threadIdx.x & 63u;
+        const uint32_t lane = tid & 63u;
         const u64 seg0 = seg - lane;
         if (lane == 0 && seg0 < g.nseg) {
             if (SMALL) {
@@ -655,21 +655,18 @@
                 }
             }
         }
-        if (MODE == 1 && a.acct && a.rows_cnt && bid == 0 && threadIdx.x == 0) atomicAdd(a.acct, *a.rows_cnt);
+        if (MODE == 1 && !WL && a.acct && a.rows_cnt && bid == 0 && tid == 0) atomicAdd(a.acct, *a.rows_cnt);
     }
 
     uint32_t live_new = (valid && on_next) ? popc(Bn | Cn) : 0u;
     if (!SMALL) live_new = group_sum(live_new, g.W);
-    if (__ballot(live_new != 0u) != 0ull && (threadIdx.x & 63u) == 0u) blk_any = 1u;
-    constexpr bool kZBlk = GS_RK_ZSKIP_BLK && TRANSITION && kBlk != 64u;
-    const u64 nz_mask = SMALL ? L.m : ~0ull;
-    if (kZBlk && __ballot(valid && ((N[0] | N[1] | N[2]) & nz_mask) != 0ull) != 0ull && (threadIdx.x & 63u) == 0u)
-        blk_nz = 1u;
+    if (__ballot(live_new != 0u) != 0ull && (tid & 63u) == 0u) blk_any = 1u;
     __syncthreads();
     const bool blk_live = blk_any != 0u;
     __builtin_amdgcn_s_setprio(1);
-    const bool zskip = kZBlk ? blk_nz == 0u
-                             : GS_RK_ZSKIP && kBlk == 64u && __ballot(valid && (N[0] | N[1] | N[2]) != 0ull) == 0ull;
+    const bool wave_nz = kBlk == 64u && __ballot(valid && (N[0] | N[1] | N[2]) != 0ull) != 0ull;
+    const bool zskip = GS_RK_ZSKIP && kBlk == 64u && !wave_nz;
+    if (kBlk == 64u && !SHARD && a.wnz && wave_nz && wave_was_a && tid == 0) a.wnz[bid] = 1u;
     if (zskip) {
     } else if (SMALL) {
         const uint32_t npu = 1u << g.lognpu;
@@ -686,7 +683,7 @@
     if (!zskip) __syncthreads();
     if (!zskip) {
         uint4 *dst4 = reinterpret_cast<uint4 *>(a.Snext + blk_base);
-        for (uint32_t i = threadIdx.x, si = s4; i < blk_v4; i += blockDim.x, si += s4d)
+        for (uint32_t i = tid, si = s4; i < blk_v4; i += kBlk, si += s4d)
             nt_store4(*reinterpret_cast<const uint4 *>(&stage[si]), &dst4[i]);
     }
     if (SHARD) {
@@ -727,6 +724,33 @@
         v.w += d_recv;
         store_stats(a.st32, a.st16, x, v);
         if (!on_next) atomicAdd(&a.offc[x], 1u);
+    }
+}
+
+template <bool SMALL, int MODE, bool SHARD, bool SEQ, bool DLV, uint32_t BLK = 256u, bool EXT = false, bool WL = false>
+__global__ __launch_bounds__(BLK, BLK == 256u ? GS_RK_MINW : GS_RK_MINW_SMALL) void round_kernel(RoundArgs a) {
+    if constexpr (WL) {
+        const uint32_t cnt = __builtin_amdgcn_readfirstlane(a.wl_cnt[a.wl_par]);
+        if (blockIdx.x == 0 && threadIdx.x == 0) {
+            if (a.wl_host) __hip_atomic_store(a.wl_host, (a.wl_tag << 32) | cnt, __ATOMIC_RELAXED, __HIP_MEMORY_SCOPE_SYSTEM);
+            atomicAdd(a.wl_total, (u64)cnt);
+            if (a.wl_acct) atomicAdd(a.wl_acct, (u64)cnt);
+        }
+        const uint32_t *list = a.wl_list;
+        for (uint32_t i = blockIdx.x; i < cnt; i += gridDim.x) {
+#if defined(__HIP_DEVICE_COMPILE__)
+            const __attribute__((address_space(4))) RoundArgs *pa =
+                (const __attribute__((address_space(4))) RoundArgs *)__builtin_amdgcn_kernarg_segment_ptr();
+            asm volatile("" : "+s"(pa));
+            const RoundArgs b = *pa;
+#else
+            const RoundArgs &b = a;
+#endif
+            round_block<SMALL, MODE, SHARD, SEQ, DLV, BLK, EXT, true>(b, __builtin_amdgcn_readfirstlane(list[i]));
+            __syncthreads();
+        }
+    } else {
+        round_block<SMALL, MODE, SHARD, SEQ, DLV, BLK, EXT, false>(a, 0u);
     }
 }
 
@@ -790,6 +814,119 @@
     return a.g.small ? launch_mode<true, false, false>(a, mode, s) : launch_mode<false, false, false>(a, mode, s);
 }
 
+constexpr uint32_t kLightThreads = 512u, kLightPer = 4u, kLightNodes = kLightThreads * kLightPer;
+__global__ __launch_bounds__(kLightThreads) void round_light(RoundArgs a) {
+    const Geometry &g = a.g;
+    __shared__ uint32_t s_cnt, s_base;
+    if (threadIdx.x == 0) s_cnt = 0u;
+    if (a.zero_buf || a.zero_rows) zero_for_build(a.zero_buf, a.zero_words, a.zero_rows, kLightThreads);
+    if (a.zero_buf2) zero_for_build(a.zero_buf2, a.zero_words2, nullptr, kLightThreads);
+    if (blockIdx.x == 0) {
+        if (threadIdx.x < kLiveSlots)
+            __hip_atomic_store(&a.live[(((a.round_new + 1u) & 1u) * kLiveSlots + threadIdx.x) * kLiveStride], 0u,
+                               __ATOMIC_RELAXED, __HIP_MEMORY_SCOPE_AGENT);
+        if (threadIdx.x == 0) {
+            a.wl_cnt[a.wl_par ^ 1u] = 0u;
+            if (a.acct && a.rows_cnt) atomicAdd(a.acct, *a.rows_cnt);
+        }
+    }
+    __syncthreads();
+    const uint32_t lw = g.logr - 6u, glog = 6u - lw;
+    const uint32_t lane = threadIdx.x & 63u, gfirst = lane & ~((1u << glog) - 1u);
+    const u64 gbits = (glog == 6u ? ~0ull : ((1ull << (1u << glog)) - 1ull)) << gfirst;
+    const u64 below = (1ull << lane) - 1ull;
+    const uint32_t x0 = blockIdx.x * kLightNodes + threadIdx.x;
+    const uint32_t serial = a.serial & kSerialMask;
+    uint32_t kf[kLightPer], tag[kLightPer], zw[kLightPer], wb[kLightPer];
+    uint4 sv[kLightPer];
+#pragma unroll
+    for (uint32_t i = 0; i < kLightPer; ++i) {
+        const uint32_t x = x0 + i * kLightThreads, xi = x < g.n ? x : 0u;
+        kf[i] = a.IN8[xi].kf;
+        tag[i] = a.SIB8[xi].tag;
+        zw[i] = reinterpret_cast<const uint32_t *>(a.zlm)[xi >> 5];
+        wb[i] = a.wnz[xi >> glog];
+        sv[i] = load_stats(a.st32, a.st16, xi);
+    }
+    uint32_t off[kLightPer], rank[kLightPer];
+    bool lead[kLightPer];
+#pragma unroll
+    for (uint32_t i = 0; i < kLightPer; ++i) {
+        const uint32_t x = x0 + i * kLightThreads;
+        const bool ok = x < g.n;
+        bool work = wb[i] != 0u || ((kf[i] >> kInSkipShift) & 7u) != 7u || (kf[i] & kInTailLive) != 0u ||
+                    (tag[i] >> 8) == serial || ((zw[i] >> (x & 31u)) & 1u) != 0u;
+        if (a.n_inj && ok) {
+            const u64 k0 = (u64)x << lw, k1 = ((u64)x + 1u) << lw;
+            uint32_t lo = 0, hi = a.n_inj;
+            while (lo < hi) {
+                const uint32_t mid = (lo + hi) >> 1;
+                if (a.inj_key[mid] < k0) lo = mid + 1; else hi = mid;
+            }
+            work |= lo < a.n_inj && a.inj_key[lo] < k1;
+        }
+        const bool wave_work = (__ballot(ok && work) & gbits) != 0ull;
+        if (ok && !wave_work) {
+            uint4 v = sv[i];
+            v.x += kf[i] & ((1u << kFirstShift) - 1u);
+            v.y += 1u;
+            store_stats(a.st32, a.st16, x, v);
+        }
+        lead[i] = ok && wave_work && lane == gfirst;
+        const u64 lb = __ballot(lead[i]);
+        rank[i] = popc(lb & below);
+        uint32_t o = 0u;
+        if (lane == 0u && lb) o = atomicAdd(&s_cnt, popc(lb));
+        off[i] = __shfl(o, 0, 64);
+    }
+    __syncthreads();
+    if (threadIdx.x == 0) s_base = s_cnt ? atomicAdd(&a.wl_cnt[a.wl_par], s_cnt) : 0u;
+    __syncthreads();
+    const uint32_t base = s_base;
+#pragma unroll
+    for (uint32_t i = 0; i < kLightPer; ++i)
+        if (lead[i]) a.wl_list[base + off[i] + rank[i]] = (x0 + i * kLightThreads) >> glog;
+}
+
+bool worklist_eligible(const RoundArgs &a, int mode) {
+    return GS_RK_ZSKIP && kRkSmallBlk == 64u && mode == 1 && !a.g.small && a.g.W <= 8u && !a.recvA && !a.Wb &&
+           !a.DR && a.zlm && a.lvm && a.cpm && a.wnz && a.wl_list && a.wl_cnt && a.wl_total && a.n_ext == 0 && !faults_on(a.f) &&
+           !a.emin && !a.eadd && !a.st16 && a.blk_off == 0 && a.blk_count == 0 && !a.blk_list &&
+           !w32_eligible(a, mode);
+}
+
+hipError_t launch_round_worklist(const RoundArgs &a, uint32_t grid, hipStream_t s) {
+    if constexpr (kRkSmallBlk == 64u) {
+        if (!worklist_eligible(a, 1) || grid == 0) return hipErrorInvalidValue;
+        hipLaunchKernelGGL(round_light, dim3((a.g.n + kLightNodes - 1u) / kLightNodes), dim3(kLightThreads), 0, s, a);
+        hipError_t err = hipGetLastError();
+        if (err != hipSuccess) return err;
+        RoundArgs h = a;
+        h.zero_buf = h.zero_buf2 = nullptr;
+        h.zero_rows = nullptr;
+        h.acct = nullptr;
+        const uint32_t blocks = (uint32_t)std::min<u64>(grid, wave_count(a.g));
+        hipLaunchKernelGGL((round_kernel<false, 1, false, false, false, 64u, false, true>), dim3(blocks), dim3(64), 0, s, h);
+        return hipGetLastError();
+    } else {
+        return hipErrorInvalidValue;
+    }
+}
+
+hipError_t worklist_resident_blocks(int device, uint32_t *blocks) {
+    *blocks = 0;
+    if constexpr (kRkSmallBlk == 64u) {
+        int per_cu = 0, cus = 0;
+        hipError_t err = hipOccupancyMaxActiveBlocksPerMultiprocessor(
+            &per_cu, round_kernel<false, 1, false, false, false, 64u, false, true>, 64, 0);
+        if (err != hipSuccess) return err;
+        err = hipDeviceGetAttribute(&cus, hipDeviceAttributeMultiprocessorCount, device);
+        if (err != hipSuccess) return err;
+        *blocks = (uint32_t)std::max(per_cu, 1) * (uint32_t)std::max(cus, 1);
+    }
+    return hipSuccess;
+}
+
 __global__ __launch_bounds__(256) void slice_apply(uint32_t *st32, const uint8_t *__restrict__ emin, uint32_t n,
                                                    uint32_t st16) {
     const uint32_t x = blockIdx.x * blockDim.x + threadIdx.x;
```

Measured after the change: 1988 billion (median of 6 runs). 2.3% higher.
